# sail-sg/EditAnything

Hardware: NVIDIA H100
Metric: 512x512 50-step SAM+ControlNet-inpaint images/sec; fused ControlNetx2+UNet+CFG+DDIM step ms (higher is better)
Workload: dtype fp16 storage / fp32 accumulate

## Files before the change

### editanything_b200/csrc/ea_gemm.cu

```cuda
#include "ea_common.cuh"
#include "ea_internal.h"

namespace ea {

static constexpr int BM = 128;
static constexpr int BK = 64;
static constexpr int GEMM_THREADS = 288;
static constexpr int W_TMA = 8;
static constexpr int EPI_WARPS = 8, EPI_THREADS = 256;
static constexpr int GEMM_SMEM_RING = 216 * 1024;
__host__ __device__ constexpr int gemm_epi_bytes(int bn) { return BM * (bn + 4) * 4 + 2 * 4096 * EPI_WARPS; }
__host__ __device__ constexpr int gemm_region_bytes(int bn, int stages) {
  return stages * (BM * BK * 2 + bn * BK * 2) > gemm_epi_bytes(bn) ? stages * (BM * BK * 2 + bn * BK * 2)
                                                                    : gemm_epi_bytes(bn);
}

struct GemmKParams {
  int M, N;
  int mode;
  int nkb_main;
  int nkb_extra;
  int cin_blocks;
  int BN, stages;
  int H, W, Bsz;
  int bw, bh, bn;
  int tiles_w, tiles_h;
  const float* bias;
  const float* rowvec;
  int rows_per_batch;
  int rowvec_ld;
  const ea_half* residual;
  long long ldr;
  ea_half* out;
  long long ldo;
  ea_half* out2;
  long long ldo2;
  float* out_f32;
  int act;
  float out_scale;
  int accumulate;
  int splits;
  int kb_per_split;
  int no_spin;
  float* ws;
  int* cnt;
  float2* rowstats_out;
  const float2* ln_stats;
  const float* ln_g;
  int ln_parts;
  float ln_inv_c, ln_eps;
  const float* row_scale;
  const char* pf[EA_GEMM_MAX_PREFETCH];
  long long pf_bytes[EA_GEMM_MAX_PREFETCH];
  int pf_ctas;
  unsigned long long b_policy;
};

static constexpr int GEMM_MAX_GROUPS = 3;
struct GemmGroup {
  CUtensorMap tmA0, tmA1, tmA2, tmA3, tmAx, tmB;
  GemmKParams p;
};
template <int NG>
struct GemmLaunch {
  GemmGroup g[NG];
};

__device__ __forceinline__ void tile_origin(const GemmKParams& p, int tm, int& n0, int& h0,
                                            int& w0) {
  int per_blk = p.tiles_w * p.tiles_h;
  int nb = tm / per_blk;
  int r = tm - nb * per_blk;
  int th = r / p.tiles_w;
  n0 = nb * p.bn;
  h0 = th * p.bh;
  w0 = (r - th * p.tiles_w) * p.bw;
}

struct RowInfo {
  long long m;
  bool ok;
  int batch;
};

__device__ __forceinline__ RowInfo row_info(const GemmKParams& p, int tm, int r) {
  RowInfo ri;
  if (p.mode == EA_GEMM_LINEAR) {
    ri.m = (long long)tm * BM + r;
    ri.ok = ri.m < p.M;
    ri.batch = p.rows_per_batch > 0 ? (int)(ri.m / p.rows_per_batch) : 0;
  } else {
    int n0, h0, w0;
    tile_origin(p, tm, n0, h0, w0);
    int dn = r / (p.bw * p.bh);
    int rr = r - dn * (p.bw * p.bh);
    int dh = rr / p.bw;
    int dw = rr - dh * p.bw;
    int n = n0 + dn, h = h0 + dh, w = w0 + dw;
    ri.ok = (n < p.Bsz) && (h < p.H) && (w < p.W);
    ri.m = ((long long)n * p.H + h) * p.W + w;
    ri.batch = n;
  }
  return ri;
}

__device__ __forceinline__ void epi_bar_sync() { asm volatile("bar.sync 1, 256;" ::: "memory"); }

__device__ __forceinline__ int ld_acquire_gpu(const int* p) {
  int v;
  asm volatile("ld.acquire.gpu.global.s32 %0, [%1];" : "=r"(v) : "l"(p) : "memory");
  return v;
}

__device__ __forceinline__ void l2_prefetch_hint(const GemmKParams& p, int cta, int lane, int lane0) {
  if (cta >= p.pf_ctas || lane < lane0) return;
  const int nl = 32 - lane0;
#pragma unroll 1
  for (int i = 0; i < EA_GEMM_MAX_PREFETCH; ++i) {
    if (p.pf[i] == nullptr) continue;
    const long long nlines = p.pf_bytes[i] >> 7;
    const char* base = p.pf[i];
#pragma unroll 4
    for (long long c = (long long)cta * nl + (lane - lane0); c < nlines; c += (long long)p.pf_ctas * nl)
      asm volatile("prefetch.global.L2 [%0];" ::"l"(base + (c << 7)));
  }
}

__device__ __forceinline__ void ln_row_stats(const GemmKParams& p, long long m, float& ln_r, float& ln_nm) {
  float s = 0.f, q = 0.f;
  const float2* base = p.ln_stats + m;
  for (int j0 = 0; j0 < p.ln_parts; j0 += 16) {
    float2 v[16];
#pragma unroll
    for (int u = 0; u < 16; ++u)
      v[u] = (j0 + u < p.ln_parts) ? __ldcg(base + (size_t)(j0 + u) * p.M) : make_float2(0.f, 0.f);
#pragma unroll
    for (int u = 0; u < 16; ++u) {
      s += v[u].x;
      q += v[u].y;
    }
  }
  const float mu = s * p.ln_inv_c;
  ln_r = rsqrtf(fmaxf(q * p.ln_inv_c - mu * mu, 0.f) + p.ln_eps);
  ln_nm = -ln_r * mu;
}

__device__ __noinline__ float act_call(float x, int act) {
  return act == EA_ACT_SILU ? silu_f(x) : gelu_erf_f(x);
}

__device__ __forceinline__ void stage_put32(uint4* stg, int lane, int half, const uint4 (&o)[4]) {
#pragma unroll
  for (int q = 0; q < 4; ++q) stg[lane * 8 + ((half * 4 + q) ^ (lane & 7))] = o[q];
}
__device__ __forceinline__ void stage_flush(const uint4* stg, int lane, ea_half* out, long long ldo,
                                            ea_half* out2, long long ldo2, long long m_mine, bool ok_mine,
                                            int col0, int pieces, int n_limit, long long lin_m0, int M) {
  __syncwarp();
  const int piece = lane & 7, rsub = lane >> 3;
  const int col = col0 + piece * 8;
  const bool col_ok = piece < pieces && col < n_limit;
  uint4 val[8];
#pragma unroll
  for (int i = 0; i < 8; ++i) {
    const int row = i * 4 + rsub;
    val[i] = stg[row * 8 + (piece ^ (row & 7))];
  }
  if (lin_m0 >= 0) {
    const long long m0 = lin_m0 + rsub;
    ea_half* ptr = out + m0 * ldo + col;
    ea_half* ptr2 = out2 ? out2 + m0 * ldo2 + col : nullptr;
    const long long step = 4 * ldo, step2 = 4 * ldo2;
#pragma unroll
    for (int i = 0; i < 8; ++i) {
      if (col_ok && m0 + 4 * i < M) {
        *reinterpret_cast<uint4*>(ptr) = val[i];
        if (ptr2) *reinterpret_cast<uint4*>(ptr2) = val[i];
      }
      ptr += step;
      if (ptr2) ptr2 += step2;
    }
  } else {
#pragma unroll
    for (int i = 0; i < 8; ++i) {
      const int row = i * 4 + rsub;
      const long long m_r = __shfl_sync(0xffffffffu, m_mine, row);
      const int ok_r = __shfl_sync(0xffffffffu, (int)ok_mine, row);
      if (ok_r && col_ok) {
        *reinterpret_cast<uint4*>(out + m_r * ldo + col) = val[i];
        if (out2) *reinterpret_cast<uint4*>(out2 + m_r * ldo2 + col) = val[i];
      }
    }
  }
  __syncwarp();
}

__device__ __forceinline__ void stage_flush32(const uint4* stg, int lane, ea_half* out, long long ldo, int col0,
                                              int n_limit, long long lin_m0, int M) {
  __syncwarp();
  const int piece = lane & 3, rsub = lane >> 2;
  const int col = col0 + piece * 8;
  const bool col_ok = col < n_limit;
  uint4 val[4];
#pragma unroll
  for (int i = 0; i < 4; ++i) {
    const int row = i * 8 + rsub;
    val[i] = stg[row * 8 + (piece ^ (row & 7))];
  }
  const long long m0 = lin_m0 + rsub;
  ea_half* ptr = out + m0 * ldo + col;
  const long long step = 8 * ldo;
#pragma unroll
  for (int i = 0; i < 4; ++i) {
    if (col_ok && m0 + 8 * i < M) *reinterpret_cast<uint4*>(ptr) = val[i];
    ptr += step;
  }
  __syncwarp();
}

__device__ __forceinline__ void residual_load64(uint4 (&rr)[8], const ea_half* residual, long long ldr,
                                                int lane, long long m_mine, bool ok_mine, int col0,
                                                int cols_left, int n_limit, long long lin_m0, int M) {
  const int piece = lane & 7, rsub = lane >> 3;
  const int col = col0 + piece * 8;
#pragma unroll
  for (int i = 0; i < 8; ++i) {
    const int row = i * 4 + rsub;
    long long m_r;
    int ok_r;
    if (lin_m0 >= 0) {
      m_r = lin_m0 + row;
      ok_r = m_r < M;
    } else {
      m_r = __shfl_sync(0xffffffffu, m_mine, row);
      ok_r = __shfl_sync(0xffffffffu, (int)ok_mine, row);
    }
    rr[i] = (ok_r && piece * 8 < cols_left && col < n_limit)
                ? __ldg(reinterpret_cast<const uint4*>(residual + m_r * ldr + col))
                : make_uint4(0, 0, 0, 0);
  }
}

__device__ __forceinline__ void epilogue_geglu32(const float* cb, int half_bn, int c, float (&fx)[32],
                                                 float (&fg)[32], uint4 (&o)[4], bool ln, float ln_r,
                                                 float ln_nm) {
  uint32_t packed[16];
#pragma unroll
  for (int j = 0; j < 32; j += 4) {
    float4 bx = *reinterpret_cast<const float4*>(cb + c + j);
    float4 bg = *reinterpret_cast<const float4*>(cb + half_bn + c + j);
    if (ln) {
      const float4 gx = *reinterpret_cast<const float4*>(cb + 256 + c + j);
      const float4 gg = *reinterpret_cast<const float4*>(cb + 256 + half_bn + c + j);
      bx.x = fmaf(ln_nm, gx.x, bx.x); bx.y = fmaf(ln_nm, gx.y, bx.y); bx.z = fmaf(ln_nm, gx.z, bx.z); bx.w = fmaf(ln_nm, gx.w, bx.w);
      bg.x = fmaf(ln_nm, gg.x, bg.x); bg.y = fmaf(ln_nm, gg.y, bg.y); bg.z = fmaf(ln_nm, gg.z, bg.z); bg.w = fmaf(ln_nm, gg.w, bg.w);
    }
    const float x0 = fmaf(fx[j], ln_r, bx.x), x1 = fmaf(fx[j + 1], ln_r, bx.y);
    const float x2 = fmaf(fx[j + 2], ln_r, bx.z), x3 = fmaf(fx[j + 3], ln_r, bx.w);
    const float g0 = fmaf(fg[j], ln_r, bg.x), g1 = fmaf(fg[j + 1], ln_r, bg.y);
    const float g2 = fmaf(fg[j + 2], ln_r, bg.z), g3 = fmaf(fg[j + 3], ln_r, bg.w);
    packed[j >> 1] = ea_pack2(x0 * gelu_erf_f(g0), x1 * gelu_erf_f(g1));
    packed[(j >> 1) + 1] = ea_pack2(x2 * gelu_erf_f(g2), x3 * gelu_erf_f(g3));
  }
#pragma unroll
  for (int q = 0; q < 4; ++q)
    o[q] = make_uint4(packed[4 * q], packed[4 * q + 1], packed[4 * q + 2], packed[4 * q + 3]);
}

__device__ __forceinline__ void epilogue_geglu32_direct(const GemmKParams& p, const RowInfo& ri, int ncol0,
                                                        int half_bn, int c, float (&fx)[32],
                                                        float (&fg)[32]) {
  const int nout0 = (ncol0 >> 1) + c;
  if (!(ri.ok && nout0 < (p.N >> 1))) return;
  uint32_t packed[16];
#pragma unroll
  for (int j = 0; j < 32; j += 2) {
    float x0 = fx[j], x1 = fx[j + 1], g0 = fg[j], g1 = fg[j + 1];
    if (p.bias) {
      x0 += __ldg(p.bias + ncol0 + c + j);
      x1 += __ldg(p.bias + ncol0 + c + j + 1);
      g0 += __ldg(p.bias + ncol0 + half_bn + c + j);
      g1 += __ldg(p.bias + ncol0 + half_bn + c + j + 1);
    }
    packed[j >> 1] = ea_pack2(x0 * act_call(g0, EA_ACT_GELU), x1 * act_call(g1, EA_ACT_GELU));
  }
  uint4* dst = reinterpret_cast<uint4*>(p.out + ri.m * p.ldo + nout0);
#pragma unroll
  for (int q = 0; q < 4; ++q)
    dst[q] = make_uint4(packed[4 * q], packed[4 * q + 1], packed[4 * q + 2], packed[4 * q + 3]);
}

__device__ __forceinline__ void epilogue_chunk32(const GemmKParams& p, const RowInfo& ri,
                                                 int n_first, float (&f)[32]) {
  if (!(ri.ok && n_first < p.N)) return;
  const long long m = ri.m;
  if (p.bias) {
#pragma unroll
    for (int j = 0; j < 32; j += 4) {
      if (n_first + j < p.N) {
        float4 b = __ldg(reinterpret_cast<const float4*>(p.bias + n_first + j));
        f[j] += b.x; f[j + 1] += b.y; f[j + 2] += b.z; f[j + 3] += b.w;
      }
    }
  }
  if (p.rowvec) {
    const float* rv = p.rowvec + (long long)ri.batch * p.rowvec_ld + n_first;
#pragma unroll
    for (int j = 0; j < 32; j += 4) {
      if (n_first + j < p.N) {
        float4 b = __ldg(reinterpret_cast<const float4*>(rv + j));
        f[j] += b.x; f[j + 1] += b.y; f[j + 2] += b.z; f[j + 3] += b.w;
      }
    }
  }
  if (p.act == EA_ACT_SILU) {
#pragma unroll
    for (int j = 0; j < 32; ++j) f[j] = act_call(f[j], EA_ACT_SILU);
  } else if (p.act == EA_ACT_GELU) {
#pragma unroll
    for (int j = 0; j < 32; ++j) f[j] = act_call(f[j], EA_ACT_GELU);
  }
  if (p.out_scale != 1.0f) {
#pragma unroll
    for (int j = 0; j < 32; ++j) f[j] *= p.out_scale;
  }
  if (p.row_scale) {
    const float rs = __ldg(p.row_scale + m);
#pragma unroll
    for (int j = 0; j < 32; ++j) f[j] *= rs;
  }
  if (p.residual) {
    const uint4* rp = reinterpret_cast<const uint4*>(p.residual + m * p.ldr + n_first);
#pragma unroll
    for (int q = 0; q < 4; ++q) {
      if (n_first + q * 8 < p.N) {
        uint4 u = __ldg(rp + q);
        float2 a = ea_unpack2(u.x), b = ea_unpack2(u.y), cc = ea_unpack2(u.z), d = ea_unpack2(u.w);
        f[q * 8 + 0] += a.x; f[q * 8 + 1] += a.y; f[q * 8 + 2] += b.x; f[q * 8 + 3] += b.y;
        f[q * 8 + 4] += cc.x; f[q * 8 + 5] += cc.y; f[q * 8 + 6] += d.x; f[q * 8 + 7] += d.y;
      }
    }
  }
  if (p.out_f32) {
    float* dst = p.out_f32 + m * p.ldo + n_first;
#pragma unroll
    for (int j = 0; j < 32; j += 4) {
      if (n_first + j < p.N) {
        float4 o = make_float4(f[j], f[j + 1], f[j + 2], f[j + 3]);
        if (p.accumulate) {
          float4 old = *reinterpret_cast<float4*>(dst + j);
          o.x += old.x; o.y += old.y; o.z += old.z; o.w += old.w;
        }
        *reinterpret_cast<float4*>(dst + j) = o;
      }
    }
    return;
  }
  uint4* dst = reinterpret_cast<uint4*>(p.out + m * p.ldo + n_first);
  if (p.accumulate) {
#pragma unroll
    for (int q = 0; q < 4; ++q) {
      if (n_first + q * 8 < p.N) {
        uint4 u = dst[q];
        float2 a = ea_unpack2(u.x), b = ea_unpack2(u.y), cc = ea_unpack2(u.z), d = ea_unpack2(u.w);
        f[q * 8 + 0] += a.x; f[q * 8 + 1] += a.y; f[q * 8 + 2] += b.x; f[q * 8 + 3] += b.y;
        f[q * 8 + 4] += cc.x; f[q * 8 + 5] += cc.y; f[q * 8 + 6] += d.x; f[q * 8 + 7] += d.y;
      }
    }
  }
  uint4* dst2 = p.out2 ? reinterpret_cast<uint4*>(p.out2 + m * p.ldo2 + n_first) : nullptr;
#pragma unroll
  for (int q = 0; q < 4; ++q) {
    if (n_first + q * 8 < p.N) {
      uint4 o = make_uint4(ea_pack2(f[q * 8 + 0], f[q * 8 + 1]), ea_pack2(f[q * 8 + 2], f[q * 8 + 3]),
                           ea_pack2(f[q * 8 + 4], f[q * 8 + 5]), ea_pack2(f[q * 8 + 6], f[q * 8 + 7]));
      dst[q] = o;
      if (dst2) dst2[q] = o;
    }
  }
}


static int encode_2d(CUtensorMap* m, const void* base, uint64_t inner, uint64_t outer,
                     uint64_t row_stride_bytes, uint32_t box_inner, uint32_t box_outer) {
  cuuint64_t dims[2] = {inner, outer};
  cuuint64_t strides[1] = {row_stride_bytes};
  cuuint32_t box[2] = {box_inner, box_outer};
  cuuint32_t estr[2] = {1, 1};
  CUresult r = ea_tmap_encode()(m, EA_TMAP_DTYPE, 2, const_cast<void*>(base), dims, strides, box,
                                estr, CU_TENSOR_MAP_INTERLEAVE_NONE, CU_TENSOR_MAP_SWIZZLE_128B,
                                CU_TENSOR_MAP_L2_PROMOTION_L2_256B,
                                CU_TENSOR_MAP_FLOAT_OOB_FILL_NONE);
  return r == CUDA_SUCCESS ? 0 : (int)r;
}

static int encode_4d(CUtensorMap* m, const void* base, const uint64_t dims_[4],
                     const uint64_t strides_bytes[3], const uint32_t box_[4]) {
  cuuint64_t dims[4] = {dims_[0], dims_[1], dims_[2], dims_[3]};
  cuuint64_t strides[3] = {strides_bytes[0], strides_bytes[1], strides_bytes[2]};
  cuuint32_t box[4] = {box_[0], box_[1], box_[2], box_[3]};
  cuuint32_t estr[4] = {1, 1, 1, 1};
  CUresult r = ea_tmap_encode()(m, EA_TMAP_DTYPE, 4, const_cast<void*>(base), dims, strides, box,
                                estr, CU_TENSOR_MAP_INTERLEAVE_NONE, CU_TENSOR_MAP_SWIZZLE_128B,
                                CU_TENSOR_MAP_L2_PROMOTION_L2_256B,
                                CU_TENSOR_MAP_FLOAT_OOB_FILL_NONE);
  return r == CUDA_SUCCESS ? 0 : (int)r;
}

static void conv_geometry(int H, int W, int& bw, int& bh, int& bn) {
  bw = 1;
  while (bw * 2 <= W && bw * 2 <= 128 && (W % (bw * 2)) == 0) bw *= 2;
  bh = 1;
  while (bh * 2 <= H && bw * bh * 2 <= 128 && (H % (bh * 2)) == 0) bh *= 2;
  bn = 128 / (bw * bh);
}

__device__ __forceinline__ void acc_ld32(const float* accs, int ld, int r, int c, uint32_t (&v)[32]) {
  const float4* src = reinterpret_cast<const float4*>(accs + (size_t)r * ld + c);
#pragma unroll
  for (int j = 0; j < 8; ++j) {
    const float4 f = src[j];
    v[4 * j] = __float_as_uint(f.x); v[4 * j + 1] = __float_as_uint(f.y);
    v[4 * j + 2] = __float_as_uint(f.z); v[4 * j + 3] = __float_as_uint(f.w);
  }
}

#define EA_GEMM_TILE()                                                             \
  const int gi = NG == 1 ? 0 : tile / tiles_per_group;                             \
  const int gtile = NG == 1 ? tile : tile - gi * tiles_per_group;                  \
  const int zsplit = gtile / mn_tiles;                                             \
  const int mn = gtile - zsplit * mn_tiles;                                        \
  const GemmGroup& GG = L.g[gi];                                                   \
  const GemmKParams& p = GG.p;                                                     \
  const int tm = mn % m_tiles, tn = mn / m_tiles;                                  \
  const int kb0 = zsplit * p.kb_per_split;                                         \
  const int kb1 = min(nkb, kb0 + p.kb_per_split);

template <int BN, int NG>
__global__ void __launch_bounds__(GEMM_THREADS, 1)
ea_gemm_kernel(const __grid_constant__ GemmLaunch<NG> L, const int tiles_per_group, const int m_tiles,
               const int n_groups) {
  const GemmKParams& p0 = L.g[0].p;
  const int n_tiles = (p0.N + BN - 1) / BN;
  const int mn_tiles = m_tiles * n_tiles;
  const int num_tiles = tiles_per_group * (NG == 1 ? 1 : n_groups);
  const int nkb = p0.nkb_main + p0.nkb_extra;
  constexpr int a_bytes = BM * BK * 2;
  constexpr int stage_bytes = a_bytes + BN * BK * 2;
  constexpr int ACC_LD = BN + 4;
  extern __shared__ __align__(1024) uint8_t smem_raw[];
  uint8_t* smem = reinterpret_cast<uint8_t*>((reinterpret_cast<uintptr_t>(smem_raw) + 1023) &
                                             ~uintptr_t(1023));
  float* accs = reinterpret_cast<float*>(smem);
  uint8_t* stg_base = smem + BM * ACC_LD * 4;
  uint64_t* full_bar = reinterpret_cast<uint64_t*>(smem + gemm_region_bytes(BN, p0.stages));
  uint64_t* empty_bar = full_bar + p0.stages;
  uint64_t* epi_done = empty_bar + p0.stages;
  float* cb = reinterpret_cast<float*>(epi_done + 2);

  pdl_launch_dependents();
  const int warp = threadIdx.x >> 5;
  const int lane = threadIdx.x & 31;

  if (warp == W_TMA && lane == 0) {
    const int g0 = NG == 1 ? 0 : min((int)blockIdx.x / tiles_per_group, n_groups - 1);
    tma_prefetch_desc(&L.g[g0].tmA0);
    tma_prefetch_desc(&L.g[g0].tmB);
    if (p0.mode == EA_GEMM_CONV_S2 || p0.mode == EA_GEMM_CONV_S2A) {
      tma_prefetch_desc(&L.g[g0].tmA1);
      tma_prefetch_desc(&L.g[g0].tmA2);
      tma_prefetch_desc(&L.g[g0].tmA3);
    }
    if (p0.nkb_extra > 0) tma_prefetch_desc(&L.g[g0].tmAx);
  }
  if (warp == W_TMA) {
    for (int g = 0; g < (NG == 1 ? 1 : n_groups); ++g) l2_prefetch_hint(L.g[g].p, (int)blockIdx.x, lane, 2);
  }
  if (warp == W_TMA && lane == 1) {
    for (int s = 0; s < p0.stages; ++s) {
      mbar_init(&full_bar[s], 1);
      mbar_init(&empty_bar[s], EPI_WARPS);
    }
    mbar_init(epi_done, EPI_WARPS);
    fence_mbar_init();
  }
  __syncthreads();

  if (warp >= EPI_WARPS) {
    pdl_wait();
    if (lane != 0) return;
    int stage = 0;
    uint32_t phase = 0;
    uint8_t* sa = smem;
    int it = 0;
    for (int tile = blockIdx.x; tile < num_tiles; tile += gridDim.x, ++it) {
      EA_GEMM_TILE()
      const CUtensorMap& tmA0 = GG.tmA0;
      const CUtensorMap& tmA1 = GG.tmA1;
      const CUtensorMap& tmA2 = GG.tmA2;
      const CUtensorMap& tmA3 = GG.tmA3;
      const CUtensorMap& tmAx = GG.tmAx;
      const CUtensorMap& tmB = GG.tmB;
      if (it > 0) mbar_wait(epi_done, (uint32_t)((it - 1) & 1));
      const int bcol = tn * BN;
      if (p.mode == EA_GEMM_LINEAR) {
        const int arow = tm * BM;
        for (int kb = kb0; kb < kb1; ++kb) {
          mbar_wait(&empty_bar[stage], phase ^ 1u);
          mbar_expect_tx(&full_bar[stage], (uint32_t)stage_bytes);
          tma_load_2d(sa, &tmA0, &full_bar[stage], kb * BK, arow);
          tma_load_2d_hint(sa + a_bytes, &tmB, &full_bar[stage], kb * BK, bcol, p.b_policy);
          sa += stage_bytes;
          if (++stage == p.stages) { stage = 0; phase ^= 1u; sa = smem; }
        }
      } else {
        int n0, h0, w0;
        tile_origin(p, tm, n0, h0, w0);
        int tap = kb0 / p.cin_blocks;
        int c0 = (kb0 - tap * p.cin_blocks) * BK;
        int kh = tap / 3, kw = tap - kh * 3;
        const int cin = p.cin_blocks * BK;
        for (int kb = kb0; kb < kb1; ++kb) {
          mbar_wait(&empty_bar[stage], phase ^ 1u);
          mbar_expect_tx(&full_bar[stage], (uint32_t)stage_bytes);
          if (kb >= p.nkb_main) {
            tma_load_4d(sa, &tmAx, &full_bar[stage], (kb - p.nkb_main) * BK, w0, h0, n0);
          } else if (p.mode == EA_GEMM_CONV_S1) {
            tma_load_4d(sa, &tmA0, &full_bar[stage], c0, w0 + kw - 1, h0 + kh - 1, n0);
          } else {
            const bool asym = p.mode == EA_GEMM_CONV_S2A;
            const int ph = asym ? (kh == 1 ? 1 : 0) : (kh == 1 ? 0 : 1);
            const int dh = asym ? (kh == 2 ? 1 : 0) : (kh == 0 ? -1 : 0);
            const int pw = asym ? (kw == 1 ? 1 : 0) : (kw == 1 ? 0 : 1);
            const int dw = asym ? (kw == 2 ? 1 : 0) : (kw == 0 ? -1 : 0);
            const int sel = ph * 2 + pw;
            const CUtensorMap* m = sel == 0 ? &tmA0 : sel == 1 ? &tmA1 : sel == 2 ? &tmA2 : &tmA3;
            tma_load_4d(sa, m, &full_bar[stage], c0, w0 + dw, h0 + dh, n0);
          }
          tma_load_2d_hint(sa + a_bytes, &tmB, &full_bar[stage], kb * BK, bcol, p.b_policy);
          c0 += BK;
          if (c0 == cin) { c0 = 0; if (++kw == 3) { kw = 0; ++kh; } }
          sa += stage_bytes;
          if (++stage == p.stages) { stage = 0; phase ^= 1u; sa = smem; }
        }
      }
    }
    return;
  }

  pdl_wait();
  const int wg = warp >> 2;
  const int wq = warp & 3;
  const int r = wq * 32 + lane;
  const int et = threadIdx.x;
  constexpr int GSTEP = 128;
  uint4* stg = reinterpret_cast<uint4*>(stg_base + warp * 4096);
  uint4* stg2 = reinterpret_cast<uint4*>(stg_base + 4096 * EPI_WARPS + warp * 4096);
  const uint32_t smem0 = smem_u32(smem);
  int stage = 0;
  uint32_t phase = 0;
  int it = 0;
  for (int tile = blockIdx.x; tile < num_tiles; tile += gridDim.x, ++it) {
    EA_GEMM_TILE()
    const bool geglu = p.act == EA_ACT_GEGLU;
    const int half_bn = BN >> 1;
    const bool has_res = p.residual != nullptr;
    const RowInfo ri = row_info(p, tm, r);
    const int ncol0 = tn * BN;
    float* cbt = cb + (it & 1) * 512;
    const long long lin_m0 = p.mode == EA_GEMM_LINEAR ? (long long)tm * BM + wq * 32 : -1;
    const int b_first = row_info(p, tm, 0).batch, b_last = row_info(p, tm, BM - 1).batch;
    const bool fast = p.splits == 1 && !geglu && !p.out_f32 && !p.accumulate && !p.row_scale && (b_last - b_first) <= 1;
    uint4 rres[8];
    const bool ln = p.ln_stats != nullptr;
    float ln_r = 1.f, ln_nm = 0.f;
    if (ln && ri.ok) ln_row_stats(p, ri.m, ln_r, ln_nm);
    if (fast) {
      for (int i = et; i < BN; i += EPI_THREADS) {
        const int col = ncol0 + i;
        float v0 = 0.f, v1 = 0.f;
        if (col < p.N) {
          const float bsum = p.bias ? __ldg(p.bias + col) : 0.f;
          v0 = bsum + (p.rowvec ? __ldg(p.rowvec + (long long)b_first * p.rowvec_ld + col) : 0.f);
          v1 = ln ? __ldg(p.ln_g + col)
                  : bsum + (p.rowvec ? __ldg(p.rowvec + (long long)b_last * p.rowvec_ld + col) : 0.f);
        }
        cbt[i] = v0;
        cbt[256 + i] = v1;
      }
      if (has_res && wg * 64 < BN)
        residual_load64(rres, p.residual, p.ldr, lane, ri.m, ri.ok, ncol0 + wg * 64, BN - wg * 64, p.N, lin_m0, p.M);
    } else if (geglu && p.splits == 1) {
      for (int i = et; i < BN; i += EPI_THREADS) {
        const bool in = ncol0 + i < p.N;
        cbt[i] = (p.bias && in) ? __ldg(p.bias + ncol0 + i) : 0.f;
        if (ln) cbt[256 + i] = in ? __ldg(p.ln_g + ncol0 + i) : 0.f;
      }
    }

    {
      float acc[BN / 2];
#pragma unroll
      for (int i = 0; i < BN / 2; ++i) acc[i] = 0.f;
      int prev = -1;
      for (int kb = kb0; kb < kb1; ++kb) {
        mbar_wait(&full_bar[stage], phase);
        const uint32_t sa = smem0 + (uint32_t)(stage * stage_bytes);
        const uint64_t da = gmma_desc_k_sw128(sa + (uint32_t)(wg * 64 * 128), 1024);
        const uint64_t db = gmma_desc_k_sw128(sa + (uint32_t)a_bytes, 1024);
        wgmma_fence();
#pragma unroll
        for (int k = 0; k < 4; ++k) Wgmma<BN>::ss(acc, da + 2 * k, db + 2 * k, 1u);
        wgmma_commit();
        wgmma_wait<1>();
        if (prev >= 0) {
          __syncwarp();
          if (lane == 0) mbar_arrive(&empty_bar[prev]);
        }
        prev = stage;
        if (++stage == p.stages) { stage = 0; phase ^= 1u; }
      }
      wgmma_wait<0>();
      wgmma_fence_regs(acc);
      if (prev >= 0) {
        __syncwarp();
        if (lane == 0) mbar_arrive(&empty_bar[prev]);
      }
      epi_bar_sync();
      const int r0 = wg * 64 + wq * 16 + (lane >> 2);
      float* d0 = accs + (size_t)r0 * ACC_LD + 2 * (lane & 3);
#pragma unroll
      for (int j = 0; j < BN / 8; ++j) {
        *reinterpret_cast<float2*>(d0 + 8 * j) = make_float2(acc[4 * j], acc[4 * j + 1]);
        *reinterpret_cast<float2*>(d0 + 8 * ACC_LD + 8 * j) = make_float2(acc[4 * j + 2], acc[4 * j + 3]);
      }
    }
    epi_bar_sync();

    if (fast) {
      const float* cbr = cbt + ((!ln && ri.batch != b_first) ? 256 : 0);
      auto next_chunk = [&](int c) { return ((c & 32) == 0 && c + 32 < BN) ? c + 32 : (c & ~63) + GSTEP; };
      for (int c = wg * 64; c < BN; c = next_chunk(c)) {
        uint32_t v[32];
        acc_ld32(accs, ACC_LD, r, c, v);
        const int n_first = ncol0 + c;
        const int half = (c >> 5) & 1;
        if (has_res && half == 0) {
          const int piece = lane & 7, rsub = lane >> 3;
#pragma unroll
          for (int i = 0; i < 8; ++i) {
            const int row = i * 4 + rsub;
            stg2[row * 8 + (piece ^ (row & 7))] = rres[i];
          }
          __syncwarp();
          if (c + GSTEP < BN)
            residual_load64(rres, p.residual, p.ldr, lane, ri.m, ri.ok, n_first + GSTEP, BN - c - GSTEP, p.N, lin_m0, p.M);
        }
        float f[32];
        if (ln) {
#pragma unroll
          for (int j = 0; j < 32; j += 4) {
            const float4 b4 = *reinterpret_cast<const float4*>(cbt + c + j);
            const float4 g4 = *reinterpret_cast<const float4*>(cbt + 256 + c + j);
            f[j] = fmaf(__uint_as_float(v[j]), ln_r, fmaf(ln_nm, g4.x, b4.x));
            f[j + 1] = fmaf(__uint_as_float(v[j + 1]), ln_r, fmaf(ln_nm, g4.y, b4.y));
            f[j + 2] = fmaf(__uint_as_float(v[j + 2]), ln_r, fmaf(ln_nm, g4.z, b4.z));
            f[j + 3] = fmaf(__uint_as_float(v[j + 3]), ln_r, fmaf(ln_nm, g4.w, b4.w));
          }
        } else {
#pragma unroll
          for (int j = 0; j < 32; j += 4) {
            const float4 b4 = *reinterpret_cast<const float4*>(cbr + c + j);
            f[j] = __uint_as_float(v[j]) + b4.x;
            f[j + 1] = __uint_as_float(v[j + 1]) + b4.y;
            f[j + 2] = __uint_as_float(v[j + 2]) + b4.z;
            f[j + 3] = __uint_as_float(v[j + 3]) + b4.w;
          }
        }
        if (p.act == EA_ACT_SILU) {
#pragma unroll
          for (int j = 0; j < 32; ++j) f[j] = act_call(f[j], EA_ACT_SILU);
        } else if (p.act == EA_ACT_GELU) {
#pragma unroll
          for (int j = 0; j < 32; ++j) f[j] = gelu_erf_f(f[j]);
        }
        if (p.out_scale != 1.0f) {
#pragma unroll
          for (int j = 0; j < 32; ++j) f[j] *= p.out_scale;
        }
#pragma unroll
        for (int q = 0; q < 4; ++q) {
          const int slot = lane * 8 + ((half * 4 + q) ^ (lane & 7));
          if (has_res) {
            const uint4 rc = stg2[slot];
            const float2 a = ea_unpack2(rc.x), b = ea_unpack2(rc.y), cc = ea_unpack2(rc.z), d = ea_unpack2(rc.w);
            f[q * 8 + 0] += a.x; f[q * 8 + 1] += a.y; f[q * 8 + 2] += b.x; f[q * 8 + 3] += b.y;
            f[q * 8 + 4] += cc.x; f[q * 8 + 5] += cc.y; f[q * 8 + 6] += d.x; f[q * 8 + 7] += d.y;
          }
          stg[slot] = make_uint4(ea_pack2(f[q * 8 + 0], f[q * 8 + 1]), ea_pack2(f[q * 8 + 2], f[q * 8 + 3]),
                                 ea_pack2(f[q * 8 + 4], f[q * 8 + 5]), ea_pack2(f[q * 8 + 6], f[q * 8 + 7]));
        }
        if (p.rowstats_out) {
          float s0 = 0.f, s1 = 0.f, q0 = 0.f, q1 = 0.f;
#pragma unroll
          for (int j = 0; j < 32; j += 2) {
            s0 += f[j]; q0 = fmaf(f[j], f[j], q0);
            s1 += f[j + 1]; q1 = fmaf(f[j + 1], f[j + 1], q1);
          }
          if (ri.ok && n_first < p.N) p.rowstats_out[(size_t)(n_first >> 5) * p.M + ri.m] = make_float2(s0 + s1, q0 + q1);
        }
        if (half == 1 || c + 32 >= BN)
          stage_flush(stg, lane, p.out, p.ldo, p.out2, p.ldo2, ri.m, ri.ok, n_first - half * 32,
                      half == 1 ? 8 : 4, p.N, lin_m0, p.M);
      }
    } else if (p.splits == 1) {
      if (geglu) {
        for (int c = wg * 32; c < half_bn; c += 64) {
          uint32_t xv[32], gv[32];
          acc_ld32(accs, ACC_LD, r, c, xv);
          acc_ld32(accs, ACC_LD, r, half_bn + c, gv);
          float fx[32], fg[32];
#pragma unroll
          for (int j = 0; j < 32; ++j) { fx[j] = __uint_as_float(xv[j]); fg[j] = __uint_as_float(gv[j]); }
          uint4 o[4];
          epilogue_geglu32(cbt, half_bn, c, fx, fg, o, ln, ln_r, ln_nm);
          stage_put32(stg, lane, 0, o);
          if (lin_m0 >= 0)
            stage_flush32(stg, lane, p.out, p.ldo, (ncol0 >> 1) + c, p.N >> 1, lin_m0, p.M);
          else
            stage_flush(stg, lane, p.out, p.ldo, nullptr, 0, ri.m, ri.ok, (ncol0 >> 1) + c, 4, p.N >> 1, lin_m0, p.M);
        }
      } else {
        for (int c = wg * 32; c < BN; c += 64) {
          uint32_t v[32];
          acc_ld32(accs, ACC_LD, r, c, v);
          float f[32];
#pragma unroll
          for (int j = 0; j < 32; ++j) f[j] = __uint_as_float(v[j]);
          epilogue_chunk32(p, ri, ncol0 + c, f);
          __syncwarp();
        }
      }
    } else {
      const int tile_id = tn * m_tiles + tm;
      float* wtile = p.ws + (size_t)tile_id * p.splits * (BM * BN);
      float* mine = wtile + (size_t)zsplit * (BM * BN);
      for (int c = wg * 32; c < BN; c += 64) {
        uint32_t v[32];
        acc_ld32(accs, ACC_LD, r, c, v);
        float4* dst = reinterpret_cast<float4*>(mine + (size_t)r * BN + c);
#pragma unroll
        for (int j = 0; j < 8; ++j)
          __stcg(dst + j, make_float4(__uint_as_float(v[4 * j]), __uint_as_float(v[4 * j + 1]),
                                      __uint_as_float(v[4 * j + 2]), __uint_as_float(v[4 * j + 3])));
      }
      __threadfence();
      epi_bar_sync();
      int* cnt = p.cnt + 2 * tile_id;
      bool take_all = false;
      volatile int* flag = reinterpret_cast<volatile int*>(cbt);
      if (p.no_spin) {
        if (et == 0) *flag = atomicAdd(cnt, 1);
        epi_bar_sync();
        take_all = *flag == p.splits - 1;
        epi_bar_sync();
      } else {
        if (et == 0) {
          atomicAdd(cnt, 1);
          uint32_t spins = 0;
          while (ld_acquire_gpu(cnt) < p.splits) {
            __nanosleep(40);
            if (++spins > (1u << 24)) { asm volatile("trap;"); }
          }
        }
        epi_bar_sync();
      }
      __threadfence();
      if (!p.no_spin || take_all) {
        const int chunks = geglu ? (half_bn >> 5) : (BN >> 5);
        const int units = BM * chunks;
        const int u0 = take_all ? 0 : (int)(((long long)units * zsplit) / p.splits);
        const int u1 = take_all ? units : (int)(((long long)units * (zsplit + 1)) / p.splits);
        const int segs = geglu ? 2 : 1;
        const int ustride = segs * 32 + 4;
        float* stage_f = accs;
        const size_t split_stride = (size_t)BM * BN;
        for (int ub = u0; ub < u1; ub += EPI_THREADS) {
          const int nu = min(EPI_THREADS, u1 - ub);
          const int nvec4 = nu * segs * 8;
          for (int idx = et; idx < nvec4; idx += EPI_THREADS) {
            const int ul = idx / (segs * 8);
            const int rem = idx - ul * (segs * 8);
            const int seg = rem >> 3, q = rem & 7;
            const int u = ub + ul;
            const int rr = u & (BM - 1);
            const int c = ((u >> 7) << 5) + seg * half_bn * (geglu ? 1 : 0);
            const float4* src = reinterpret_cast<const float4*>(wtile + (size_t)rr * BN + c) + q;
            float4 acc = make_float4(0.f, 0.f, 0.f, 0.f);
            int sidx = 0;
            for (; sidx + 4 <= p.splits; sidx += 4) {
              float4 v0 = __ldcg(src + (size_t)(sidx + 0) * (split_stride >> 2));
              float4 v1 = __ldcg(src + (size_t)(sidx + 1) * (split_stride >> 2));
              float4 v2 = __ldcg(src + (size_t)(sidx + 2) * (split_stride >> 2));
              float4 v3 = __ldcg(src + (size_t)(sidx + 3) * (split_stride >> 2));
              acc.x += v0.x; acc.y += v0.y; acc.z += v0.z; acc.w += v0.w;
              acc.x += v1.x; acc.y += v1.y; acc.z += v1.z; acc.w += v1.w;
              acc.x += v2.x; acc.y += v2.y; acc.z += v2.z; acc.w += v2.w;
              acc.x += v3.x; acc.y += v3.y; acc.z += v3.z; acc.w += v3.w;
            }
            for (; sidx < p.splits; ++sidx) {
              float4 v0 = __ldcg(src + (size_t)sidx * (split_stride >> 2));
              acc.x += v0.x; acc.y += v0.y; acc.z += v0.z; acc.w += v0.w;
            }
            *reinterpret_cast<float4*>(stage_f + ul * ustride + seg * 32 + q * 4) = acc;
          }
          epi_bar_sync();
          if (et < nu) {
            const int u = ub + et;
            const int rr = u & (BM - 1);
            const int c = (u >> 7) << 5;
            RowInfo r2 = row_info(p, tm, rr);
            const float4* sp = reinterpret_cast<const float4*>(stage_f + et * ustride);
            float f[32];
#pragma unroll
            for (int j = 0; j < 8; ++j) {
              float4 v = sp[j];
              f[4 * j] = v.x; f[4 * j + 1] = v.y; f[4 * j + 2] = v.z; f[4 * j + 3] = v.w;
            }
            if (geglu) {
              float fg[32];
#pragma unroll
              for (int j = 0; j < 8; ++j) {
                float4 v = sp[8 + j];
                fg[4 * j] = v.x; fg[4 * j + 1] = v.y; fg[4 * j + 2] = v.z; fg[4 * j + 3] = v.w;
              }
              epilogue_geglu32_direct(p, r2, ncol0, half_bn, c, f, fg);
            } else {
              epilogue_chunk32(p, r2, ncol0 + c, f);
            }
          }
          epi_bar_sync();
        }
        epi_bar_sync();
        if (et == 0) {
          if (take_all) {
            cnt[0] = 0;
          } else {
            int old = atomicAdd(cnt + 1, 1);
            if (old == p.splits - 1) {
              cnt[0] = 0;
              cnt[1] = 0;
            }
          }
        }
      }
    }
    fence_proxy_async();
    __syncwarp();
    if (lane == 0) mbar_arrive(epi_done);
  }
}
#undef EA_GEMM_TILE

struct GemmPlan { int BN, stages, splits, kbps, occ; double cost; };

static constexpr double PL_LAT = 2100.0, PL_SM_CAP = 57.0, PL_L2 = 3000.0, PL_HBM = 1900.0;
static constexpr double PL_SPLIT_COL = 8.0, PL_SPLIT_FIX = 7000.0;
static constexpr double PL_START = 3800.0, PL_EPI = 50.0, PL_EPI_RES = 21.0;
static constexpr int GEMM_BN[3] = {128, 64, 32};

static GemmPlan plan_gemm(int mt, int N, int nkb, int act, long long ws_floats, int n_sm, bool has_res = false,
                          int groups = 1) {
  const double epi_col = (PL_EPI + (has_res ? PL_EPI_RES : 0.0)) * (act == EA_ACT_GEGLU ? 0.84 : 1.0);
  GemmPlan best = {0, 0, 1, nkb, 1, 1e30};
  for (int BN : GEMM_BN) {
    if (act == EA_ACT_GEGLU && BN != 128) continue;
    if (BN > 32 && N <= BN - 32) continue;
    const int nt = (N + BN - 1) / BN;
    const long long tiles = (long long)mt * nt * groups;
    const int stage_bytes = BM * BK * 2 + BN * BK * 2;
    int st = GEMM_SMEM_RING / stage_bytes;
    if (st > 8) st = 8;
    if (st > nkb) st = nkb < 2 ? 2 : nkb;
    const long long slots = n_sm;
    for (int pass = 0; pass < 2; ++pass) {
      int splits = 1, kbps = nkb;
      if (pass == 1) {
        if (tiles >= slots || nkb < 8) break;
        int s_max = (int)(slots / tiles);
        if (s_max > nkb / 4) s_max = nkb / 4;
        if (s_max < 2) break;
        kbps = (nkb + s_max - 1) / s_max;
        splits = (nkb + kbps - 1) / kbps;
        if (splits < 2) break;
        if (tiles > 2048 || tiles * splits * (long long)(BM * BN) > ws_floats) break;
      }
      const long long ctas = tiles * splits;
      const long long waves = (ctas + slots - 1) / slots;
      const long long conc = ctas < slots ? ctas : slots;
      const double t_mma = 4.0 * BN;
      const double t_sm = (double)stage_bytes / PL_SM_CAP;
      const double a_bytes = BM * BK * 2.0, b_bytes = BN * BK * 2.0;
      const double hbm_frac = 1.0 / (double)mt;
      const double t_chip = (double)conc * (a_bytes / PL_L2 + b_bytes * hbm_frac / PL_HBM +
                                            b_bytes * (1.0 - hbm_frac) / PL_L2);
      const double t_lat = PL_LAT / st;
      double t_kb = t_mma;
      if (t_sm > t_kb) t_kb = t_sm;
      if (t_chip > t_kb) t_kb = t_chip;
      if (t_lat > t_kb) t_kb = t_lat;
      double cost;
      if (splits == 1) {
        cost = (double)waves * (PL_START + kbps * t_kb + epi_col * BN);
      } else {
        cost = (double)waves * (PL_START + kbps * t_kb + PL_SPLIT_COL * BN) + PL_SPLIT_FIX +
               3.0 * (BM * BN * 4.0) / 25.0 + 150.0 * splits;
      }
      if (cost < best.cost) best = {BN, st, splits, kbps, 1, cost};
    }
  }
  return best;
}

static int sm_count() { return ea_sm_count(); }

}

using namespace ea;

extern "C" int ea_gemm_plan(int m_tiles, int N, int k_blocks, int act, long long workspace_bytes,
                            int n_sm, int* out5) {
  if (!out5 || m_tiles <= 0 || N <= 0 || k_blocks <= 0) return EA_ERR_ARG;
  const long long ws_floats = workspace_bytes > 65536 ? (workspace_bytes - 65536) / 4 : 0;
  GemmPlan pl = plan_gemm(m_tiles, N, k_blocks, act, ws_floats, n_sm > 0 ? n_sm : 132);
  out5[0] = pl.BN; out5[1] = pl.stages; out5[2] = pl.splits; out5[3] = pl.kbps;
  out5[4] = pl.occ;
  return pl.BN ? EA_OK : EA_ERR_SHAPE;
}

struct GemmShape {
  int m_tiles, nkb;
  long long Ktot;
  bool ln_any;
};

static int gemm_fill_group(const ea_gemm_args* a, GemmGroup& G, GemmShape& sh) {
  if (!a || !a->a || !a->w || (!a->out && !a->out_f32)) return EA_ERR_ARG;
  if (a->mode < 0 || a->mode > EA_GEMM_CONV_S2A) return EA_ERR_ARG;
  if (a->N <= 0 || a->M <= 0) return EA_ERR_ARG;
  if (a->N % 8 != 0) return EA_ERR_SHAPE;
  GemmKParams& p = G.p;
  memset(&p, 0, sizeof(p));
  p.M = a->M;
  p.N = a->N;
  p.mode = a->mode;
  p.bias = a->bias;
  p.rowvec = a->rowvec;
  p.rows_per_batch = a->rows_per_batch;
  p.rowvec_ld = a->rowvec_ld;
  p.residual = reinterpret_cast<const ea_half*>(a->residual);
  p.ldr = a->ldr;
  p.out = reinterpret_cast<ea_half*>(a->out);
  p.ldo = a->ldo;
  p.out2 = reinterpret_cast<ea_half*>(a->out2);
  p.ldo2 = a->ldo2;
  p.out_f32 = a->out_f32;
  p.act = a->act;
  p.out_scale = a->out_scale;
  p.accumulate = a->accumulate;
  p.row_scale = a->row_scale;
  for (int i = 0; i < EA_GEMM_MAX_PREFETCH; ++i) {
    p.pf[i] = reinterpret_cast<const char*>(a->prefetch[i]);
    p.pf_bytes[i] = a->prefetch[i] ? (a->prefetch_bytes[i] & ~15LL) : 0;
  }
  p.pf_ctas = 0;
  p.b_policy = 0x12F0000000000000ull;
  if (a->row_scale && (a->act == EA_ACT_GEGLU || a->rowstats_out || a->ln_stats)) return EA_ERR_ARG;
  sh.ln_any = a->rowstats_out || a->ln_stats;
  if (sh.ln_any) {
    if (a->mode != EA_GEMM_LINEAR || a->rowvec || a->out_f32 || a->accumulate) return EA_ERR_ARG;
    if (a->rowstats_out && (a->N % 32 != 0 || a->act == EA_ACT_GEGLU)) return EA_ERR_SHAPE;
    if (a->ln_stats && (!a->ln_g || a->ln_parts <= 0 || a->K != a->ln_parts * 32)) return EA_ERR_ARG;
    p.rowstats_out = reinterpret_cast<float2*>(a->rowstats_out);
    p.ln_stats = reinterpret_cast<const float2*>(a->ln_stats);
    p.ln_g = a->ln_g;
    p.ln_parts = a->ln_parts;
    p.ln_inv_c = a->ln_stats ? 1.0f / (float)a->K : 0.f;
    p.ln_eps = a->ln_eps;
  }
  if (p.ldo % 8 != 0 || (p.residual && p.ldr % 8 != 0) || (p.out2 && p.ldo2 % 8 != 0))
    return EA_ERR_SHAPE;

  CUtensorMap* tmA[4] = {&G.tmA0, &G.tmA1, &G.tmA2, &G.tmA3};
  if (a->mode == EA_GEMM_LINEAR) {
    if (a->K % 8 != 0 || a->lda % 8 != 0) return EA_ERR_SHAPE;
    p.nkb_main = (a->K + BK - 1) / BK;
    p.nkb_extra = 0;
    p.cin_blocks = 1;
    sh.m_tiles = (a->M + BM - 1) / BM;
    sh.Ktot = a->K;
    if (encode_2d(tmA[0], a->a, (uint64_t)a->K, (uint64_t)a->M, (uint64_t)a->lda * 2, BK, BM))
      return EA_ERR_TMAP;
    G.tmA1 = G.tmA2 = G.tmA3 = G.tmA0;
    G.tmAx = G.tmA0;
  } else {
    const int H = a->H, W = a->W, B = a->Bsz, C = a->Cin;
    if (C % 64 != 0 || H <= 0 || W <= 0 || B <= 0) return EA_ERR_SHAPE;
    if ((long long)B * H * W != a->M) return EA_ERR_SHAPE;
    p.H = H; p.W = W; p.Bsz = B;
    conv_geometry(H, W, p.bw, p.bh, p.bn);
    p.tiles_w = W / p.bw;
    p.tiles_h = H / p.bh;
    p.cin_blocks = C / 64;
    p.nkb_main = 9 * p.cin_blocks;
    p.nkb_extra = 0;
    sh.m_tiles = ((B + p.bn - 1) / p.bn) * p.tiles_w * p.tiles_h;
    sh.Ktot = 9LL * C;
    const long long lda = a->lda > 0 ? a->lda : C;
    uint32_t box[4] = {64, (uint32_t)p.bw, (uint32_t)p.bh, (uint32_t)p.bn};
    if (a->mode == EA_GEMM_CONV_S1) {
      uint64_t dims[4] = {(uint64_t)C, (uint64_t)W, (uint64_t)H, (uint64_t)B};
      uint64_t st[3] = {(uint64_t)lda * 2, (uint64_t)lda * W * 2, (uint64_t)lda * W * H * 2};
      if (encode_4d(tmA[0], a->a, dims, st, box)) return EA_ERR_TMAP;
      G.tmA1 = G.tmA2 = G.tmA3 = G.tmA0;
    } else {
      const int Hin = 2 * H, Win = 2 * W;
      for (int ph = 0; ph < 2; ++ph)
        for (int pw = 0; pw < 2; ++pw) {
          const ea_half* base =
              reinterpret_cast<const ea_half*>(a->a) + ((long long)ph * Win + pw) * lda;
          uint64_t dims[4] = {(uint64_t)C, (uint64_t)W, (uint64_t)H, (uint64_t)B};
          uint64_t st[3] = {(uint64_t)lda * 2 * 2, (uint64_t)lda * Win * 2 * 2,
                            (uint64_t)lda * Win * Hin * 2};
          if (encode_4d(tmA[ph * 2 + pw], base, dims, st, box)) return EA_ERR_TMAP;
        }
    }
    G.tmAx = G.tmA0;
    if (a->a_extra) {
      if (a->mode != EA_GEMM_CONV_S1 || a->Cin_extra % 64 != 0) return EA_ERR_SHAPE;
      const long long ldx = a->ld_extra > 0 ? a->ld_extra : a->Cin_extra;
      uint64_t dims[4] = {(uint64_t)a->Cin_extra, (uint64_t)W, (uint64_t)H, (uint64_t)B};
      uint64_t st[3] = {(uint64_t)ldx * 2, (uint64_t)ldx * W * 2, (uint64_t)ldx * W * H * 2};
      if (encode_4d(&G.tmAx, a->a_extra, dims, st, box)) return EA_ERR_TMAP;
      p.nkb_extra = a->Cin_extra / 64;
      sh.Ktot += a->Cin_extra;
    }
  }
  sh.nkb = p.nkb_main + p.nkb_extra;
  return EA_OK;
}

static bool gemm_same_problem(const ea_gemm_args* a, const ea_gemm_args* b) {
  return a->mode == b->mode && a->M == b->M && a->N == b->N && a->K == b->K && a->Bsz == b->Bsz && a->H == b->H &&
         a->W == b->W && a->Cin == b->Cin && a->Cin_extra == b->Cin_extra && (!a->a_extra) == (!b->a_extra) &&
         a->act == b->act && a->accumulate == b->accumulate && (!a->out_f32) == (!b->out_f32) &&
         (!a->row_scale) == (!b->row_scale) &&
         (!a->rowvec) == (!b->rowvec) && a->rows_per_batch == b->rows_per_batch &&
         (!a->rowstats_out) == (!b->rowstats_out) && (!a->ln_stats) == (!b->ln_stats) && a->ln_parts == b->ln_parts &&
         a->force_bn == b->force_bn && a->force_stages == b->force_stages && a->force_splits == b->force_splits &&
         a->force_2cta == b->force_2cta && a->no_spin == b->no_spin && a->force_persistent == b->force_persistent;
}

template <typename K>
static int set_max_smem(K kernel, int bytes, int& cached) {
  if (bytes > cached) {
    const cudaError_t e = cudaFuncSetAttribute(kernel, cudaFuncAttributeMaxDynamicSharedMemorySize, bytes);
    if (e != cudaSuccess) return ea_cuda_fail(e, "ea_gemm: cudaFuncSetAttribute(MaxDynamicSharedMemorySize)");
    cached = bytes;
  }
  return EA_OK;
}

template <int BN, int NG>
static cudaError_t launch_gemm(const GemmLaunch<NG>& L, int grid, int smem_bytes, int tiles_per_group, int m_tiles,
                               int n_groups, cudaStream_t stream, int& rc) {
  static int cache[EA_MAX_DEV];
  if ((rc = set_max_smem(ea_gemm_kernel<BN, NG>, smem_bytes, cache[ea_dev()]))) return cudaSuccess;
  return ea_launch(ea_gemm_kernel<BN, NG>, dim3((unsigned)grid), dim3(GEMM_THREADS), (size_t)smem_bytes, stream, L,
                   tiles_per_group, m_tiles, n_groups);
}

template <int NG>
static cudaError_t launch_gemm_bn(int BN, const GemmLaunch<NG>& L, int grid, int smem_bytes, int tiles_per_group,
                                  int m_tiles, int n_groups, cudaStream_t stream, int& rc) {
  switch (BN) {
    case 32: return launch_gemm<32, NG>(L, grid, smem_bytes, tiles_per_group, m_tiles, n_groups, stream, rc);
    case 64: return launch_gemm<64, NG>(L, grid, smem_bytes, tiles_per_group, m_tiles, n_groups, stream, rc);
    case 128: return launch_gemm<128, NG>(L, grid, smem_bytes, tiles_per_group, m_tiles, n_groups, stream, rc);
    default: return launch_gemm<256, NG>(L, grid, smem_bytes, tiles_per_group, m_tiles, n_groups, stream, rc);
  }
}

extern "C" int ea_gemm_grouped(const ea_gemm_args* args, int n_groups, void* stream_) {
  cudaStream_t stream = reinterpret_cast<cudaStream_t>(stream_);
  if (!args || n_groups < 1 || n_groups > GEMM_MAX_GROUPS) return EA_ERR_ARG;
  const ea_gemm_args* a = &args[0];
  static GemmLaunch<GEMM_MAX_GROUPS> L;
  GemmShape sh0;
  memset(&L, 0, sizeof(L));
  for (int g = 0; g < n_groups; ++g) {
    GemmShape shg;
    if (g > 0 && !gemm_same_problem(a, &args[g])) return EA_ERR_ARG;
    const int rc = gemm_fill_group(&args[g], L.g[g], g == 0 ? sh0 : shg);
    if (rc != EA_OK) return rc;
  }
  const int m_tiles = sh0.m_tiles, nkb = sh0.nkb;
  const bool ln_any = sh0.ln_any;
  const int G = n_groups;
  const long long ws_floats =
      (a->workspace && a->workspace_bytes > 65536 && !ln_any) ? (a->workspace_bytes - 65536) / 4 : 0;
  const bool persist = a->force_persistent > 0;
  const bool has_res = a->residual != nullptr;
  GemmPlan plan = plan_gemm(m_tiles, a->N, nkb, a->act, persist ? 0 : ws_floats, sm_count(), has_res, G);
  if (a->force_bn > 0 || a->force_stages > 0 || a->force_splits > 0) {
    if (a->force_bn > 0) plan.BN = a->force_bn;
    const int sb = BM * BK * 2 + plan.BN * BK * 2;
    if (a->force_bn > 0) plan.stages = plan.BN <= 128 ? 3 : 4;
    if (a->force_stages > 0) plan.stages = a->force_stages;
    if (plan.stages * sb > GEMM_SMEM_RING) plan.stages = GEMM_SMEM_RING / sb;
    if (plan.stages > nkb) plan.stages = nkb < 2 ? 2 : nkb;
    if (a->force_bn > 0 || a->force_splits > 0) { plan.splits = 1; plan.kbps = nkb; }
    if (a->force_splits > 1 && !persist) {
      plan.kbps = (nkb + a->force_splits - 1) / a->force_splits;
      plan.splits = (nkb + plan.kbps - 1) / plan.kbps;
    }
  }
  if (ln_any && plan.splits > 1) return EA_ERR_ARG;
  const int BN = plan.BN;
  if (BN != 32 && BN != 64 && BN != 128 && BN != 256) return EA_ERR_SHAPE;
  if (a->act == EA_ACT_GEGLU && (a->N % 128 != 0 || BN != 128)) return EA_ERR_SHAPE;
  const int n_tiles = (a->N + BN - 1) / BN;
  const long long tiles = (long long)m_tiles * n_tiles;
  if (plan.splits > 1 &&
      (!ws_floats || tiles * G > 8192 || tiles * G * plan.splits * (long long)(BM * BN) > ws_floats))
    return EA_ERR_SHAPE;
  if (plan.splits > 1 && !a->no_spin && tiles * G * plan.splits > (long long)sm_count()) return EA_ERR_SHAPE;

  int stages = plan.stages;
  if (stages > 8) stages = 8;
  if (stages < 2) stages = 2;
  const int smem_bytes = gemm_region_bytes(BN, stages) + (2 * stages + 2) * 8 + 2 * 2 * 256 * 4 + 1024;
  const long long tiles_per_group = tiles * plan.splits;
  for (int g = 0; g < G; ++g) {
    GemmKParams& p = L.g[g].p;
    const ea_gemm_args* ag = &args[g];
    p.BN = BN;
    p.stages = stages;
    p.splits = plan.splits;
    p.kb_per_split = plan.kbps;
    p.no_spin = a->no_spin;
    if (p.splits > 1) {
      p.cnt = reinterpret_cast<int*>(a->workspace) + 2 * g * tiles;
      p.ws = reinterpret_cast<float*>(reinterpret_cast<char*>(a->workspace) + 65536) +
             (size_t)g * tiles * p.splits * (BM * BN);
    }
    const long long ldw = ag->ldw > 0 ? ag->ldw : sh0.Ktot;
    if (ldw % 8 != 0) return EA_ERR_SHAPE;
    if (encode_2d(&L.g[g].tmB, ag->w, (uint64_t)sh0.Ktot, (uint64_t)ag->N, (uint64_t)ldw * 2, BK, (uint32_t)BN))
      return EA_ERR_TMAP;
  }
  if (m_tiles > 64)
    for (int g = 0; g < G; ++g) L.g[g].p.b_policy = 0ull;
  const long long total = tiles_per_group * G;
  const int grid = (int)(persist && total > sm_count() ? sm_count() : total);
  for (int g = 0; g < G; ++g)
    L.g[g].p.pf_ctas = grid < sm_count() ? grid : sm_count();

  cudaError_t le;
  int rc = EA_OK;
  if (G == 1) {
    GemmLaunch<1> L1;
    L1.g[0] = L.g[0];
    le = launch_gemm_bn<1>(BN, L1, grid, smem_bytes, (int)tiles_per_group, m_tiles, G, stream, rc);
  } else {
    le = launch_gemm_bn<GEMM_MAX_GROUPS>(BN, L, grid, smem_bytes, (int)tiles_per_group, m_tiles, G, stream, rc);
  }
  if (rc) return rc;
  ea_count_launch();
  if (le != cudaSuccess) return ea_cuda_fail(le, "ea_gemm: kernel launch");
  const cudaError_t ke = cudaGetLastError();
  return ke == cudaSuccess ? 0 : ea_cuda_fail(ke, "ea_gemm: after the kernel launch");
}

extern "C" int ea_gemm(const ea_gemm_args* a, void* stream) { return ea_gemm_grouped(a, 1, stream); }
```

Measured before the change: 1.618.

## Warp-specialize GEMM with separate MMA and epilogue warpgroups and register rebalancing

Splits the GEMM kernel into a producer warp, dedicated MMA warps and separate epilogue warps, so the epilogue of one tile can overlap the mainloop of the next. Accumulator staging moves to its own shared-memory region with acc_full/acc_empty barriers, and setmaxnreg redistributes registers between roles. Small-BN and short-K tiles also default to a persistent grid. The cost is fewer pipeline stages, because the ring and the epilogue buffer now share shared memory, plus more threads per CTA, which can cost registers in the MMA warps.

```diff
diff --git a/editanything_b200/csrc/ea_gemm.cu b/editanything_b200/csrc/ea_gemm.cu
--- a/editanything_b200/csrc/ea_gemm.cu
+++ b/editanything_b200/csrc/ea_gemm.cu
@@ -5,14 +5,43 @@
 
 static constexpr int BM = 128;
 static constexpr int BK = 64;
-static constexpr int GEMM_THREADS = 288;
-static constexpr int W_TMA = 8;
+static constexpr int GEMM_THREADS = 640;
+static constexpr int W_TMA = 16;
+static constexpr int MMA_WARPS = 8;
 static constexpr int EPI_WARPS = 8, EPI_THREADS = 256;
+static constexpr int GEMM_LAUNCH_REGS = (65536 / GEMM_THREADS) & ~7;
+template <int BN, bool SPLIT>
+struct GemmRegs {
+  static constexpr bool split_epi = SPLIT;
+  static constexpr int producer = 48;
+  static constexpr int mma = split_epi ? BN / 2 + 32 : 192;
+  static constexpr int epi = split_epi ? ((5 * GEMM_LAUNCH_REGS - producer - 2 * mma) / 2) & ~7 : 24;
+  static_assert(producer + 2 * mma + 2 * epi <= 5 * GEMM_LAUNCH_REGS, "setmaxnreg budgets exceed the launch");
+};
+template <int R> __device__ __forceinline__ void setmaxnreg() {
+  if constexpr (R > GEMM_LAUNCH_REGS)
+    asm volatile("setmaxnreg.inc.sync.aligned.u32 %0;" ::"n"(R));
+  else if constexpr (R < GEMM_LAUNCH_REGS)
+    asm volatile("setmaxnreg.dec.sync.aligned.u32 %0;" ::"n"(R));
+}
 static constexpr int GEMM_SMEM_RING = 216 * 1024;
-__host__ __device__ constexpr int gemm_epi_bytes(int bn) { return BM * (bn + 4) * 4 + 2 * 4096 * EPI_WARPS; }
-__host__ __device__ constexpr int gemm_region_bytes(int bn, int stages) {
-  return stages * (BM * BK * 2 + bn * BK * 2) > gemm_epi_bytes(bn) ? stages * (BM * BK * 2 + bn * BK * 2)
-                                                                    : gemm_epi_bytes(bn);
+static constexpr int GEMM_SMEM_MAX = 227 * 1024;
+__host__ __device__ constexpr int gemm_epi_bytes(int bn) { return BM * (bn + 4) * 4 + 4096 * EPI_WARPS; }
+__host__ __device__ constexpr int gemm_ring_bytes(int bn, int stages) { return stages * (BM * BK * 2 + bn * BK * 2); }
+__host__ __device__ constexpr int gemm_region_bytes(int bn, int stages, bool split) {
+  return split ? gemm_ring_bytes(bn, stages) + gemm_epi_bytes(bn)
+               : (gemm_ring_bytes(bn, stages) > gemm_epi_bytes(bn) ? gemm_ring_bytes(bn, stages) : gemm_epi_bytes(bn));
+}
+__host__ __device__ constexpr int gemm_smem_bytes(int bn, int stages, bool split) {
+  return gemm_region_bytes(bn, stages, split) + (2 * stages + 2) * 8 + 2 * 2 * 256 * 4 + 1024;
+}
+static constexpr int GEMM_SPLIT_EPI_MAX_KB = 20;
+static bool gemm_split_epi(int bn, int kb_per_tile, int splits) {
+  return bn < 128 || (bn == 128 && splits == 1 && kb_per_tile <= GEMM_SPLIT_EPI_MAX_KB);
+}
+static int gemm_fit_stages(int bn, int stages, bool split) {
+  while (stages > 2 && gemm_smem_bytes(bn, stages, split) > GEMM_SMEM_MAX) --stages;
+  return stages;
 }
 
 struct GemmKParams {
@@ -436,10 +465,276 @@
   const int kb0 = zsplit * p.kb_per_split;                                         \
   const int kb1 = min(nkb, kb0 + p.kb_per_split);
 
-template <int BN, int NG>
+template <int BN, typename AccReady>
+__device__ __forceinline__ void gemm_epilogue(const GemmKParams& p, int tm, int tn, int zsplit, int m_tiles,
+                                              float* cbt, float* accs, uint4* stg, int wg, int wq, int lane, int et,
+                                              AccReady&& acc_ready) {
+  constexpr int ACC_LD = BN + 4;
+  const int r = wq * 32 + lane;
+  constexpr int GSTEP = 128;
+  const bool geglu = p.act == EA_ACT_GEGLU;
+  const int half_bn = BN >> 1;
+  const bool has_res = p.residual != nullptr;
+  const RowInfo ri = row_info(p, tm, r);
+  const int ncol0 = tn * BN;
+  const long long lin_m0 = p.mode == EA_GEMM_LINEAR ? (long long)tm * BM + wq * 32 : -1;
+  const int b_first = row_info(p, tm, 0).batch, b_last = row_info(p, tm, BM - 1).batch;
+  const bool fast = p.splits == 1 && !geglu && !p.out_f32 && !p.accumulate && !p.row_scale && (b_last - b_first) <= 1;
+  uint4 rres[8];
+  const bool ln = p.ln_stats != nullptr;
+  float ln_r = 1.f, ln_nm = 0.f;
+  if (ln && ri.ok) ln_row_stats(p, ri.m, ln_r, ln_nm);
+  if (fast) {
+    for (int i = et; i < BN; i += EPI_THREADS) {
+      const int col = ncol0 + i;
+      float v0 = 0.f, v1 = 0.f;
+      if (col < p.N) {
+        const float bsum = p.bias ? __ldg(p.bias + col) : 0.f;
+        v0 = bsum + (p.rowvec ? __ldg(p.rowvec + (long long)b_first * p.rowvec_ld + col) : 0.f);
+        v1 = ln ? __ldg(p.ln_g + col)
+                : bsum + (p.rowvec ? __ldg(p.rowvec + (long long)b_last * p.rowvec_ld + col) : 0.f);
+      }
+      cbt[i] = v0;
+      cbt[256 + i] = v1;
+    }
+    if (has_res && wg * 64 < BN)
+      residual_load64(rres, p.residual, p.ldr, lane, ri.m, ri.ok, ncol0 + wg * 64, BN - wg * 64, p.N, lin_m0, p.M);
+  } else if (geglu && p.splits == 1) {
+    for (int i = et; i < BN; i += EPI_THREADS) {
+      const bool in = ncol0 + i < p.N;
+      cbt[i] = (p.bias && in) ? __ldg(p.bias + ncol0 + i) : 0.f;
+      if (ln) cbt[256 + i] = in ? __ldg(p.ln_g + ncol0 + i) : 0.f;
+    }
+  }
+
+  acc_ready();
+  epi_bar_sync();
+
+  if (fast) {
+    const float* cbr = cbt + ((!ln && ri.batch != b_first) ? 256 : 0);
+    auto next_chunk = [&](int c) { return ((c & 32) == 0 && c + 32 < BN) ? c + 32 : (c & ~63) + GSTEP; };
+    for (int c = wg * 64; c < BN; c = next_chunk(c)) {
+      uint32_t v[32];
+      acc_ld32(accs, ACC_LD, r, c, v);
+      const int n_first = ncol0 + c;
+      const int half = (c >> 5) & 1;
+      if (has_res && half == 0) {
+        const int piece = lane & 7, rsub = lane >> 3;
+#pragma unroll
+        for (int i = 0; i < 8; ++i) {
+          const int row = i * 4 + rsub;
+          stg[row * 8 + (piece ^ (row & 7))] = rres[i];
+        }
+        __syncwarp();
+        if (c + GSTEP < BN)
+          residual_load64(rres, p.residual, p.ldr, lane, ri.m, ri.ok, n_first + GSTEP, BN - c - GSTEP, p.N, lin_m0, p.M);
+      }
+      float f[32];
+      if (ln) {
+#pragma unroll
+        for (int j = 0; j < 32; j += 4) {
+          const float4 b4 = *reinterpret_cast<const float4*>(cbt + c + j);
+          const float4 g4 = *reinterpret_cast<const float4*>(cbt + 256 + c + j);
+          f[j] = fmaf(__uint_as_float(v[j]), ln_r, fmaf(ln_nm, g4.x, b4.x));
+          f[j + 1] = fmaf(__uint_as_float(v[j + 1]), ln_r, fmaf(ln_nm, g4.y, b4.y));
+          f[j + 2] = fmaf(__uint_as_float(v[j + 2]), ln_r, fmaf(ln_nm, g4.z, b4.z));
+          f[j + 3] = fmaf(__uint_as_float(v[j + 3]), ln_r, fmaf(ln_nm, g4.w, b4.w));
+        }
+      } else {
+#pragma unroll
+        for (int j = 0; j < 32; j += 4) {
+          const float4 b4 = *reinterpret_cast<const float4*>(cbr + c + j);
+          f[j] = __uint_as_float(v[j]) + b4.x;
+          f[j + 1] = __uint_as_float(v[j + 1]) + b4.y;
+          f[j + 2] = __uint_as_float(v[j + 2]) + b4.z;
+          f[j + 3] = __uint_as_float(v[j + 3]) + b4.w;
+        }
+      }
+      if (p.act == EA_ACT_SILU) {
+#pragma unroll
+        for (int j = 0; j < 32; ++j) f[j] = act_call(f[j], EA_ACT_SILU);
+      } else if (p.act == EA_ACT_GELU) {
+#pragma unroll
+        for (int j = 0; j < 32; ++j) f[j] = gelu_erf_f(f[j]);
+      }
+      if (p.out_scale != 1.0f) {
+#pragma unroll
+        for (int j = 0; j < 32; ++j) f[j] *= p.out_scale;
+      }
+#pragma unroll
+      for (int q = 0; q < 4; ++q) {
+        const int slot = lane * 8 + ((half * 4 + q) ^ (lane & 7));
+        if (has_res) {
+          const uint4 rc = stg[slot];
+          const float2 a = ea_unpack2(rc.x), b = ea_unpack2(rc.y), cc = ea_unpack2(rc.z), d = ea_unpack2(rc.w);
+          f[q * 8 + 0] += a.x; f[q * 8 + 1] += a.y; f[q * 8 + 2] += b.x; f[q * 8 + 3] += b.y;
+          f[q * 8 + 4] += cc.x; f[q * 8 + 5] += cc.y; f[q * 8 + 6] += d.x; f[q * 8 + 7] += d.y;
+        }
+        stg[slot] = make_uint4(ea_pack2(f[q * 8 + 0], f[q * 8 + 1]), ea_pack2(f[q * 8 + 2], f[q * 8 + 3]),
+                               ea_pack2(f[q * 8 + 4], f[q * 8 + 5]), ea_pack2(f[q * 8 + 6], f[q * 8 + 7]));
+      }
+      if (p.rowstats_out) {
+        float s0 = 0.f, s1 = 0.f, q0 = 0.f, q1 = 0.f;
+#pragma unroll
+        for (int j = 0; j < 32; j += 2) {
+          s0 += f[j]; q0 = fmaf(f[j], f[j], q0);
+          s1 += f[j + 1]; q1 = fmaf(f[j + 1], f[j + 1], q1);
+        }
+        if (ri.ok && n_first < p.N) p.rowstats_out[(size_t)(n_first >> 5) * p.M + ri.m] = make_float2(s0 + s1, q0 + q1);
+      }
+      if (half == 1 || c + 32 >= BN)
+        stage_flush(stg, lane, p.out, p.ldo, p.out2, p.ldo2, ri.m, ri.ok, n_first - half * 32,
+                    half == 1 ? 8 : 4, p.N, lin_m0, p.M);
+    }
+  } else if (p.splits == 1) {
+    if (geglu) {
+      for (int c = wg * 32; c < half_bn; c += 64) {
+        uint32_t xv[32], gv[32];
+        acc_ld32(accs, ACC_LD, r, c, xv);
+        acc_ld32(accs, ACC_LD, r, half_bn + c, gv);
+        float fx[32], fg[32];
+#pragma unroll
+        for (int j = 0; j < 32; ++j) { fx[j] = __uint_as_float(xv[j]); fg[j] = __uint_as_float(gv[j]); }
+        uint4 o[4];
+        epilogue_geglu32(cbt, half_bn, c, fx, fg, o, ln, ln_r, ln_nm);
+        stage_put32(stg, lane, 0, o);
+        if (lin_m0 >= 0)
+          stage_flush32(stg, lane, p.out, p.ldo, (ncol0 >> 1) + c, p.N >> 1, lin_m0, p.M);
+        else
+          stage_flush(stg, lane, p.out, p.ldo, nullptr, 0, ri.m, ri.ok, (ncol0 >> 1) + c, 4, p.N >> 1, lin_m0, p.M);
+      }
+    } else {
+      for (int c = wg * 32; c < BN; c += 64) {
+        uint32_t v[32];
+        acc_ld32(accs, ACC_LD, r, c, v);
+        float f[32];
+#pragma unroll
+        for (int j = 0; j < 32; ++j) f[j] = __uint_as_float(v[j]);
+        epilogue_chunk32(p, ri, ncol0 + c, f);
+        __syncwarp();
+      }
+    }
+  } else {
+    const int tile_id = tn * m_tiles + tm;
+    float* wtile = p.ws + (size_t)tile_id * p.splits * (BM * BN);
+    float* mine = wtile + (size_t)zsplit * (BM * BN);
+    for (int c = wg * 32; c < BN; c += 64) {
+      uint32_t v[32];
+      acc_ld32(accs, ACC_LD, r, c, v);
+      float4* dst = reinterpret_cast<float4*>(mine + (size_t)r * BN + c);
+#pragma unroll
+      for (int j = 0; j < 8; ++j)
+        __stcg(dst + j, make_float4(__uint_as_float(v[4 * j]), __uint_as_float(v[4 * j + 1]),
+                                    __uint_as_float(v[4 * j + 2]), __uint_as_float(v[4 * j + 3])));
+    }
+    __threadfence();
+    epi_bar_sync();
+    int* cnt = p.cnt + 2 * tile_id;
+    bool take_all = false;
+    volatile int* flag = reinterpret_cast<volatile int*>(cbt);
+    if (p.no_spin) {
+      if (et == 0) *flag = atomicAdd(cnt, 1);
+      epi_bar_sync();
+      take_all = *flag == p.splits - 1;
+      epi_bar_sync();
+    } else {
+      if (et == 0) {
+        atomicAdd(cnt, 1);
+        uint32_t spins = 0;
+        while (ld_acquire_gpu(cnt) < p.splits) {
+          __nanosleep(40);
+          if (++spins > (1u << 24)) { asm volatile("trap;"); }
+        }
+      }
+      epi_bar_sync();
+    }
+    __threadfence();
+    if (!p.no_spin || take_all) {
+      const int chunks = geglu ? (half_bn >> 5) : (BN >> 5);
+      const int units = BM * chunks;
+      const int u0 = take_all ? 0 : (int)(((long long)units * zsplit) / p.splits);
+      const int u1 = take_all ? units : (int)(((long long)units * (zsplit + 1)) / p.splits);
+      const int segs = geglu ? 2 : 1;
+      const int ustride = segs * 32 + 4;
+      float* stage_f = accs;
+      const size_t split_stride = (size_t)BM * BN;
+      for (int ub = u0; ub < u1; ub += EPI_THREADS) {
+        const int nu = min(EPI_THREADS, u1 - ub);
+        const int nvec4 = nu * segs * 8;
+        for (int idx = et; idx < nvec4; idx += EPI_THREADS) {
+          const int ul = idx / (segs * 8);
+          const int rem = idx - ul * (segs * 8);
+          const int seg = rem >> 3, q = rem & 7;
+          const int u = ub + ul;
+          const int rr = u & (BM - 1);
+          const int c = ((u >> 7) << 5) + seg * half_bn * (geglu ? 1 : 0);
+          const float4* src = reinterpret_cast<const float4*>(wtile + (size_t)rr * BN + c) + q;
+          float4 acc = make_float4(0.f, 0.f, 0.f, 0.f);
+          int sidx = 0;
+          for (; sidx + 4 <= p.splits; sidx += 4) {
+            float4 v0 = __ldcg(src + (size_t)(sidx + 0) * (split_stride >> 2));
+            float4 v1 = __ldcg(src + (size_t)(sidx + 1) * (split_stride >> 2));
+            float4 v2 = __ldcg(src + (size_t)(sidx + 2) * (split_stride >> 2));
+            float4 v3 = __ldcg(src + (size_t)(sidx + 3) * (split_stride >> 2));
+            acc.x += v0.x; acc.y += v0.y; acc.z += v0.z; acc.w += v0.w;
+            acc.x += v1.x; acc.y += v1.y; acc.z += v1.z; acc.w += v1.w;
+            acc.x += v2.x; acc.y += v2.y; acc.z += v2.z; acc.w += v2.w;
+            acc.x += v3.x; acc.y += v3.y; acc.z += v3.z; acc.w += v3.w;
+          }
+          for (; sidx < p.splits; ++sidx) {
+            float4 v0 = __ldcg(src + (size_t)sidx * (split_stride >> 2));
+            acc.x += v0.x; acc.y += v0.y; acc.z += v0.z; acc.w += v0.w;
+          }
+          *reinterpret_cast<float4*>(stage_f + ul * ustride + seg * 32 + q * 4) = acc;
+        }
+        epi_bar_sync();
+        if (et < nu) {
+          const int u = ub + et;
+          const int rr = u & (BM - 1);
+          const int c = (u >> 7) << 5;
+          RowInfo r2 = row_info(p, tm, rr);
+          const float4* sp = reinterpret_cast<const float4*>(stage_f + et * ustride);
+          float f[32];
+#pragma unroll
+          for (int j = 0; j < 8; ++j) {
+            float4 v = sp[j];
+            f[4 * j] = v.x; f[4 * j + 1] = v.y; f[4 * j + 2] = v.z; f[4 * j + 3] = v.w;
+          }
+          if (geglu) {
+            float fg[32];
+#pragma unroll
+            for (int j = 0; j < 8; ++j) {
+              float4 v = sp[8 + j];
+              fg[4 * j] = v.x; fg[4 * j + 1] = v.y; fg[4 * j + 2] = v.z; fg[4 * j + 3] = v.w;
+            }
+            epilogue_geglu32_direct(p, r2, ncol0, half_bn, c, f, fg);
+          } else {
+            epilogue_chunk32(p, r2, ncol0 + c, f);
+          }
+        }
+        epi_bar_sync();
+      }
+      epi_bar_sync();
+      if (et == 0) {
+        if (take_all) {
+          cnt[0] = 0;
+        } else {
+          int old = atomicAdd(cnt + 1, 1);
+          if (old == p.splits - 1) {
+            cnt[0] = 0;
+            cnt[1] = 0;
+          }
+        }
+      }
+    }
+  }
+}
+
+template <int BN, int NG, bool SPLIT>
 __global__ void __launch_bounds__(GEMM_THREADS, 1)
 ea_gemm_kernel(const __grid_constant__ GemmLaunch<NG> L, const int tiles_per_group, const int m_tiles,
                const int n_groups) {
+  using R = GemmRegs<BN, SPLIT>;
   const GemmKParams& p0 = L.g[0].p;
   const int n_tiles = (p0.N + BN - 1) / BN;
   const int mn_tiles = m_tiles * n_tiles;
@@ -451,12 +746,13 @@
   extern __shared__ __align__(1024) uint8_t smem_raw[];
   uint8_t* smem = reinterpret_cast<uint8_t*>((reinterpret_cast<uintptr_t>(smem_raw) + 1023) &
                                              ~uintptr_t(1023));
-  float* accs = reinterpret_cast<float*>(smem);
-  uint8_t* stg_base = smem + BM * ACC_LD * 4;
-  uint64_t* full_bar = reinterpret_cast<uint64_t*>(smem + gemm_region_bytes(BN, p0.stages));
+  float* accs = reinterpret_cast<float*>(R::split_epi ? smem + gemm_ring_bytes(BN, p0.stages) : smem);
+  uint8_t* stg_base = reinterpret_cast<uint8_t*>(accs) + BM * ACC_LD * 4;
+  uint64_t* full_bar = reinterpret_cast<uint64_t*>(smem + gemm_region_bytes(BN, p0.stages, SPLIT));
   uint64_t* empty_bar = full_bar + p0.stages;
-  uint64_t* epi_done = empty_bar + p0.stages;
-  float* cb = reinterpret_cast<float*>(epi_done + 2);
+  uint64_t* acc_full = empty_bar + p0.stages;
+  uint64_t* acc_empty = acc_full + 1;
+  float* cb = reinterpret_cast<float*>(acc_empty + 1);
 
   pdl_launch_dependents();
   const int warp = threadIdx.x >> 5;
@@ -479,16 +775,18 @@
   if (warp == W_TMA && lane == 1) {
     for (int s = 0; s < p0.stages; ++s) {
       mbar_init(&full_bar[s], 1);
-      mbar_init(&empty_bar[s], EPI_WARPS);
-    }
-    mbar_init(epi_done, EPI_WARPS);
+      mbar_init(&empty_bar[s], MMA_WARPS);
+    }
+    mbar_init(acc_full, MMA_WARPS);
+    mbar_init(acc_empty, R::split_epi ? EPI_WARPS : MMA_WARPS);
     fence_mbar_init();
   }
   __syncthreads();
 
-  if (warp >= EPI_WARPS) {
+  if (warp >= W_TMA) {
+    setmaxnreg<R::producer>();
     pdl_wait();
-    if (lane != 0) return;
+    if (warp != W_TMA || lane != 0) return;
     int stage = 0;
     uint32_t phase = 0;
     uint8_t* sa = smem;
@@ -501,7 +799,7 @@
       const CUtensorMap& tmA3 = GG.tmA3;
       const CUtensorMap& tmAx = GG.tmAx;
       const CUtensorMap& tmB = GG.tmB;
-      if (it > 0) mbar_wait(epi_done, (uint32_t)((it - 1) & 1));
+      if (!R::split_epi && it > 0) mbar_wait(acc_empty, (uint32_t)((it - 1) & 1));
       const int bcol = tn * BN;
       if (p.mode == EA_GEMM_LINEAR) {
         const int arow = tm * BM;
@@ -548,57 +846,38 @@
     return;
   }
 
+  if (warp < EPI_WARPS) {
+    if constexpr (!R::split_epi) {
+      setmaxnreg<R::epi>();
+      return;
+    } else {
+      setmaxnreg<R::epi>();
+      pdl_wait();
+      int it = 0;
+      for (int tile = blockIdx.x; tile < num_tiles; tile += gridDim.x, ++it) {
+        EA_GEMM_TILE()
+        (void)kb0; (void)kb1;
+        gemm_epilogue<BN>(p, tm, tn, zsplit, m_tiles, cb + (it & 1) * 512, accs,
+                          reinterpret_cast<uint4*>(stg_base + warp * 4096), warp >> 2, warp & 3, lane, threadIdx.x,
+                          [&] { mbar_wait(acc_full, (uint32_t)(it & 1)); });
+        __syncwarp();
+        if (lane == 0) mbar_arrive(acc_empty);
+      }
+      return;
+    }
+  }
+
+  setmaxnreg<R::mma>();
   pdl_wait();
-  const int wg = warp >> 2;
+  const int wg = (warp >> 2) - 2;
   const int wq = warp & 3;
-  const int r = wq * 32 + lane;
-  const int et = threadIdx.x;
-  constexpr int GSTEP = 128;
-  uint4* stg = reinterpret_cast<uint4*>(stg_base + warp * 4096);
-  uint4* stg2 = reinterpret_cast<uint4*>(stg_base + 4096 * EPI_WARPS + warp * 4096);
   const uint32_t smem0 = smem_u32(smem);
   int stage = 0;
   uint32_t phase = 0;
   int it = 0;
   for (int tile = blockIdx.x; tile < num_tiles; tile += gridDim.x, ++it) {
     EA_GEMM_TILE()
-    const bool geglu = p.act == EA_ACT_GEGLU;
-    const int half_bn = BN >> 1;
-    const bool has_res = p.residual != nullptr;
-    const RowInfo ri = row_info(p, tm, r);
-    const int ncol0 = tn * BN;
-    float* cbt = cb + (it & 1) * 512;
-    const long long lin_m0 = p.mode == EA_GEMM_LINEAR ? (long long)tm * BM + wq * 32 : -1;
-    const int b_first = row_info(p, tm, 0).batch, b_last = row_info(p, tm, BM - 1).batch;
-    const bool fast = p.splits == 1 && !geglu && !p.out_f32 && !p.accumulate && !p.row_scale && (b_last - b_first) <= 1;
-    uint4 rres[8];
-    const bool ln = p.ln_stats != nullptr;
-    float ln_r = 1.f, ln_nm = 0.f;
-    if (ln && ri.ok) ln_row_stats(p, ri.m, ln_r, ln_nm);
-    if (fast) {
-      for (int i = et; i < BN; i += EPI_THREADS) {
-        const int col = ncol0 + i;
-        float v0 = 0.f, v1 = 0.f;
-        if (col < p.N) {
-          const float bsum = p.bias ? __ldg(p.bias + col) : 0.f;
-          v0 = bsum + (p.rowvec ? __ldg(p.rowvec + (long long)b_first * p.rowvec_ld + col) : 0.f);
-          v1 = ln ? __ldg(p.ln_g + col)
-                  : bsum + (p.rowvec ? __ldg(p.rowvec + (long long)b_last * p.rowvec_ld + col) : 0.f);
-        }
-        cbt[i] = v0;
-        cbt[256 + i] = v1;
-      }
-      if (has_res && wg * 64 < BN)
-        residual_load64(rres, p.residual, p.ldr, lane, ri.m, ri.ok, ncol0 + wg * 64, BN - wg * 64, p.N, lin_m0, p.M);
-    } else if (geglu && p.splits == 1) {
-      for (int i = et; i < BN; i += EPI_THREADS) {
-        const bool in = ncol0 + i < p.N;
-        cbt[i] = (p.bias && in) ? __ldg(p.bias + ncol0 + i) : 0.f;
-        if (ln) cbt[256 + i] = in ? __ldg(p.ln_g + ncol0 + i) : 0.f;
-      }
-    }
-
-    {
+    auto mma_tile = [&] {
       float acc[BN / 2];
 #pragma unroll
       for (int i = 0; i < BN / 2; ++i) acc[i] = 0.f;
@@ -610,7 +889,14 @@
         const uint64_t db = gmma_desc_k_sw128(sa + (uint32_t)a_bytes, 1024);
         wgmma_fence();
 #pragma unroll
-        for (int k = 0; k < 4; ++k) Wgmma<BN>::ss(acc, da + 2 * k, db + 2 * k, 1u);
+        for (int k = 0; k < 4; ++k) {
+          if constexpr (BN == 256) {
+            Wgmma<128>::ss(*reinterpret_cast<float(*)[64]>(acc), da + 2 * k, db + 2 * k, 1u);
+            Wgmma<128>::ss(*reinterpret_cast<float(*)[64]>(acc + 64), da + 2 * k, db + (128 * 128 >> 4) + 2 * k, 1u);
+          } else {
+            Wgmma<BN>::ss(acc, da + 2 * k, db + 2 * k, 1u);
+          }
+        }
         wgmma_commit();
         wgmma_wait<1>();
         if (prev >= 0) {
@@ -626,7 +912,11 @@
         __syncwarp();
         if (lane == 0) mbar_arrive(&empty_bar[prev]);
       }
-      epi_bar_sync();
+      if constexpr (R::split_epi) {
+        mbar_wait(acc_empty, (uint32_t)((it & 1) ^ 1));
+      } else {
+        epi_bar_sync();
+      }
       const int r0 = wg * 64 + wq * 16 + (lane >> 2);
       float* d0 = accs + (size_t)r0 * ACC_LD + 2 * (lane & 3);
 #pragma unroll
@@ -634,230 +924,19 @@
         *reinterpret_cast<float2*>(d0 + 8 * j) = make_float2(acc[4 * j], acc[4 * j + 1]);
         *reinterpret_cast<float2*>(d0 + 8 * ACC_LD + 8 * j) = make_float2(acc[4 * j + 2], acc[4 * j + 3]);
       }
-    }
-    epi_bar_sync();
-
-    if (fast) {
-      const float* cbr = cbt + ((!ln && ri.batch != b_first) ? 256 : 0);
-      auto next_chunk = [&](int c) { return ((c & 32) == 0 && c + 32 < BN) ? c + 32 : (c & ~63) + GSTEP; };
-      for (int c = wg * 64; c < BN; c = next_chunk(c)) {
-        uint32_t v[32];
-        acc_ld32(accs, ACC_LD, r, c, v);
-        const int n_first = ncol0 + c;
-        const int half = (c >> 5) & 1;
-        if (has_res && half == 0) {
-          const int piece = lane & 7, rsub = lane >> 3;
-#pragma unroll
-          for (int i = 0; i < 8; ++i) {
-            const int row = i * 4 + rsub;
-            stg2[row * 8 + (piece ^ (row & 7))] = rres[i];
-          }
-          __syncwarp();
-          if (c + GSTEP < BN)
-            residual_load64(rres, p.residual, p.ldr, lane, ri.m, ri.ok, n_first + GSTEP, BN - c - GSTEP, p.N, lin_m0, p.M);
-        }
-        float f[32];
-        if (ln) {
-#pragma unroll
-          for (int j = 0; j < 32; j += 4) {
-            const float4 b4 = *reinterpret_cast<const float4*>(cbt + c + j);
-            const float4 g4 = *reinterpret_cast<const float4*>(cbt + 256 + c + j);
-            f[j] = fmaf(__uint_as_float(v[j]), ln_r, fmaf(ln_nm, g4.x, b4.x));
-            f[j + 1] = fmaf(__uint_as_float(v[j + 1]), ln_r, fmaf(ln_nm, g4.y, b4.y));
-            f[j + 2] = fmaf(__uint_as_float(v[j + 2]), ln_r, fmaf(ln_nm, g4.z, b4.z));
-            f[j + 3] = fmaf(__uint_as_float(v[j + 3]), ln_r, fmaf(ln_nm, g4.w, b4.w));
-          }
-        } else {
-#pragma unroll
-          for (int j = 0; j < 32; j += 4) {
-            const float4 b4 = *reinterpret_cast<const float4*>(cbr + c + j);
-            f[j] = __uint_as_float(v[j]) + b4.x;
-            f[j + 1] = __uint_as_float(v[j + 1]) + b4.y;
-            f[j + 2] = __uint_as_float(v[j + 2]) + b4.z;
-            f[j + 3] = __uint_as_float(v[j + 3]) + b4.w;
-          }
-        }
-        if (p.act == EA_ACT_SILU) {
-#pragma unroll
-          for (int j = 0; j < 32; ++j) f[j] = act_call(f[j], EA_ACT_SILU);
-        } else if (p.act == EA_ACT_GELU) {
-#pragma unroll
-          for (int j = 0; j < 32; ++j) f[j] = gelu_erf_f(f[j]);
-        }
-        if (p.out_scale != 1.0f) {
-#pragma unroll
-          for (int j = 0; j < 32; ++j) f[j] *= p.out_scale;
-        }
-#pragma unroll
-        for (int q = 0; q < 4; ++q) {
-          const int slot = lane * 8 + ((half * 4 + q) ^ (lane & 7));
-          if (has_res) {
-            const uint4 rc = stg2[slot];
-            const float2 a = ea_unpack2(rc.x), b = ea_unpack2(rc.y), cc = ea_unpack2(rc.z), d = ea_unpack2(rc.w);
-            f[q * 8 + 0] += a.x; f[q * 8 + 1] += a.y; f[q * 8 + 2] += b.x; f[q * 8 + 3] += b.y;
-            f[q * 8 + 4] += cc.x; f[q * 8 + 5] += cc.y; f[q * 8 + 6] += d.x; f[q * 8 + 7] += d.y;
-          }
-          stg[slot] = make_uint4(ea_pack2(f[q * 8 + 0], f[q * 8 + 1]), ea_pack2(f[q * 8 + 2], f[q * 8 + 3]),
-                                 ea_pack2(f[q * 8 + 4], f[q * 8 + 5]), ea_pack2(f[q * 8 + 6], f[q * 8 + 7]));
-        }
-        if (p.rowstats_out) {
-          float s0 = 0.f, s1 = 0.f, q0 = 0.f, q1 = 0.f;
-#pragma unroll
-          for (int j = 0; j < 32; j += 2) {
-            s0 += f[j]; q0 = fmaf(f[j], f[j], q0);
-            s1 += f[j + 1]; q1 = fmaf(f[j + 1], f[j + 1], q1);
-          }
-          if (ri.ok && n_first < p.N) p.rowstats_out[(size_t)(n_first >> 5) * p.M + ri.m] = make_float2(s0 + s1, q0 + q1);
-        }
-        if (half == 1 || c + 32 >= BN)
-          stage_flush(stg, lane, p.out, p.ldo, p.out2, p.ldo2, ri.m, ri.ok, n_first - half * 32,
-                      half == 1 ? 8 : 4, p.N, lin_m0, p.M);
-      }
-    } else if (p.splits == 1) {
-      if (geglu) {
-        for (int c = wg * 32; c < half_bn; c += 64) {
-          uint32_t xv[32], gv[32];
-          acc_ld32(accs, ACC_LD, r, c, xv);
-          acc_ld32(accs, ACC_LD, r, half_bn + c, gv);
-          float fx[32], fg[32];
-#pragma unroll
-          for (int j = 0; j < 32; ++j) { fx[j] = __uint_as_float(xv[j]); fg[j] = __uint_as_float(gv[j]); }
-          uint4 o[4];
-          epilogue_geglu32(cbt, half_bn, c, fx, fg, o, ln, ln_r, ln_nm);
-          stage_put32(stg, lane, 0, o);
-          if (lin_m0 >= 0)
-            stage_flush32(stg, lane, p.out, p.ldo, (ncol0 >> 1) + c, p.N >> 1, lin_m0, p.M);
-          else
-            stage_flush(stg, lane, p.out, p.ldo, nullptr, 0, ri.m, ri.ok, (ncol0 >> 1) + c, 4, p.N >> 1, lin_m0, p.M);
-        }
-      } else {
-        for (int c = wg * 32; c < BN; c += 64) {
-          uint32_t v[32];
-          acc_ld32(accs, ACC_LD, r, c, v);
-          float f[32];
-#pragma unroll
-          for (int j = 0; j < 32; ++j) f[j] = __uint_as_float(v[j]);
-          epilogue_chunk32(p, ri, ncol0 + c, f);
-          __syncwarp();
-        }
-      }
+    };
+    if constexpr (R::split_epi) {
+      mma_tile();
+      __syncwarp();
+      if (lane == 0) mbar_arrive(acc_full);
     } else {
-      const int tile_id = tn * m_tiles + tm;
-      float* wtile = p.ws + (size_t)tile_id * p.splits * (BM * BN);
-      float* mine = wtile + (size_t)zsplit * (BM * BN);
-      for (int c = wg * 32; c < BN; c += 64) {
-        uint32_t v[32];
-        acc_ld32(accs, ACC_LD, r, c, v);
-        float4* dst = reinterpret_cast<float4*>(mine + (size_t)r * BN + c);
-#pragma unroll
-        for (int j = 0; j < 8; ++j)
-          __stcg(dst + j, make_float4(__uint_as_float(v[4 * j]), __uint_as_float(v[4 * j + 1]),
-                                      __uint_as_float(v[4 * j + 2]), __uint_as_float(v[4 * j + 3])));
-      }
-      __threadfence();
-      epi_bar_sync();
-      int* cnt = p.cnt + 2 * tile_id;
-      bool take_all = false;
-      volatile int* flag = reinterpret_cast<volatile int*>(cbt);
-      if (p.no_spin) {
-        if (et == 0) *flag = atomicAdd(cnt, 1);
-        epi_bar_sync();
-        take_all = *flag == p.splits - 1;
-        epi_bar_sync();
-      } else {
-        if (et == 0) {
-          atomicAdd(cnt, 1);
-          uint32_t spins = 0;
-          while (ld_acquire_gpu(cnt) < p.splits) {
-            __nanosleep(40);
-            if (++spins > (1u << 24)) { asm volatile("trap;"); }
-          }
-        }
-        epi_bar_sync();
-      }
-      __threadfence();
-      if (!p.no_spin || take_all) {
-        const int chunks = geglu ? (half_bn >> 5) : (BN >> 5);
-        const int units = BM * chunks;
-        const int u0 = take_all ? 0 : (int)(((long long)units * zsplit) / p.splits);
-        const int u1 = take_all ? units : (int)(((long long)units * (zsplit + 1)) / p.splits);
-        const int segs = geglu ? 2 : 1;
-        const int ustride = segs * 32 + 4;
-        float* stage_f = accs;
-        const size_t split_stride = (size_t)BM * BN;
-        for (int ub = u0; ub < u1; ub += EPI_THREADS) {
-          const int nu = min(EPI_THREADS, u1 - ub);
-          const int nvec4 = nu * segs * 8;
-          for (int idx = et; idx < nvec4; idx += EPI_THREADS) {
-            const int ul = idx / (segs * 8);
-            const int rem = idx - ul * (segs * 8);
-            const int seg = rem >> 3, q = rem & 7;
-            const int u = ub + ul;
-            const int rr = u & (BM - 1);
-            const int c = ((u >> 7) << 5) + seg * half_bn * (geglu ? 1 : 0);
-            const float4* src = reinterpret_cast<const float4*>(wtile + (size_t)rr * BN + c) + q;
-            float4 acc = make_float4(0.f, 0.f, 0.f, 0.f);
-            int sidx = 0;
-            for (; sidx + 4 <= p.splits; sidx += 4) {
-              float4 v0 = __ldcg(src + (size_t)(sidx + 0) * (split_stride >> 2));
-              float4 v1 = __ldcg(src + (size_t)(sidx + 1) * (split_stride >> 2));
-              float4 v2 = __ldcg(src + (size_t)(sidx + 2) * (split_stride >> 2));
-              float4 v3 = __ldcg(src + (size_t)(sidx + 3) * (split_stride >> 2));
-              acc.x += v0.x; acc.y += v0.y; acc.z += v0.z; acc.w += v0.w;
-              acc.x += v1.x; acc.y += v1.y; acc.z += v1.z; acc.w += v1.w;
-              acc.x += v2.x; acc.y += v2.y; acc.z += v2.z; acc.w += v2.w;
-              acc.x += v3.x; acc.y += v3.y; acc.z += v3.z; acc.w += v3.w;
-            }
-            for (; sidx < p.splits; ++sidx) {
-              float4 v0 = __ldcg(src + (size_t)sidx * (split_stride >> 2));
-              acc.x += v0.x; acc.y += v0.y; acc.z += v0.z; acc.w += v0.w;
-            }
-            *reinterpret_cast<float4*>(stage_f + ul * ustride + seg * 32 + q * 4) = acc;
-          }
-          epi_bar_sync();
-          if (et < nu) {
-            const int u = ub + et;
-            const int rr = u & (BM - 1);
-            const int c = (u >> 7) << 5;
-            RowInfo r2 = row_info(p, tm, rr);
-            const float4* sp = reinterpret_cast<const float4*>(stage_f + et * ustride);
-            float f[32];
-#pragma unroll
-            for (int j = 0; j < 8; ++j) {
-              float4 v = sp[j];
-              f[4 * j] = v.x; f[4 * j + 1] = v.y; f[4 * j + 2] = v.z; f[4 * j + 3] = v.w;
-            }
-            if (geglu) {
-              float fg[32];
-#pragma unroll
-              for (int j = 0; j < 8; ++j) {
-                float4 v = sp[8 + j];
-                fg[4 * j] = v.x; fg[4 * j + 1] = v.y; fg[4 * j + 2] = v.z; fg[4 * j + 3] = v.w;
-              }
-              epilogue_geglu32_direct(p, r2, ncol0, half_bn, c, f, fg);
-            } else {
-              epilogue_chunk32(p, r2, ncol0 + c, f);
-            }
-          }
-          epi_bar_sync();
-        }
-        epi_bar_sync();
-        if (et == 0) {
-          if (take_all) {
-            cnt[0] = 0;
-          } else {
-            int old = atomicAdd(cnt + 1, 1);
-            if (old == p.splits - 1) {
-              cnt[0] = 0;
-              cnt[1] = 0;
-            }
-          }
-        }
-      }
-    }
-    fence_proxy_async();
-    __syncwarp();
-    if (lane == 0) mbar_arrive(epi_done);
+      gemm_epilogue<BN>(p, tm, tn, zsplit, m_tiles, cb + (it & 1) * 512, accs,
+                        reinterpret_cast<uint4*>(stg_base + (warp - EPI_WARPS) * 4096), wg, wq, lane,
+                        threadIdx.x - EPI_THREADS, mma_tile);
+      fence_proxy_async();
+      __syncwarp();
+      if (lane == 0) mbar_arrive(acc_empty);
+    }
   }
 }
 #undef EA_GEMM_TILE
@@ -916,7 +995,8 @@
         cost = (double)waves * (PL_START + kbps * t_kb + PL_SPLIT_COL * BN) + PL_SPLIT_FIX +
                3.0 * (BM * BN * 4.0) / 25.0 + 150.0 * splits;
       }
-      if (cost < best.cost) best = {BN, st, splits, kbps, 1, cost};
+      if (cost < best.cost)
+        best = {BN, gemm_fit_stages(BN, st, gemm_split_epi(BN, kbps, splits)), splits, kbps, 1, cost};
     }
   }
   return best;
@@ -1071,23 +1151,25 @@
   return EA_OK;
 }
 
-template <int BN, int NG>
+template <int BN, int NG, bool SPLIT>
 static cudaError_t launch_gemm(const GemmLaunch<NG>& L, int grid, int smem_bytes, int tiles_per_group, int m_tiles,
                                int n_groups, cudaStream_t stream, int& rc) {
   static int cache[EA_MAX_DEV];
-  if ((rc = set_max_smem(ea_gemm_kernel<BN, NG>, smem_bytes, cache[ea_dev()]))) return cudaSuccess;
-  return ea_launch(ea_gemm_kernel<BN, NG>, dim3((unsigned)grid), dim3(GEMM_THREADS), (size_t)smem_bytes, stream, L,
-                   tiles_per_group, m_tiles, n_groups);
+  if ((rc = set_max_smem(ea_gemm_kernel<BN, NG, SPLIT>, smem_bytes, cache[ea_dev()]))) return cudaSuccess;
+  return ea_launch(ea_gemm_kernel<BN, NG, SPLIT>, dim3((unsigned)grid), dim3(GEMM_THREADS), (size_t)smem_bytes, stream,
+                   L, tiles_per_group, m_tiles, n_groups);
 }
 
 template <int NG>
-static cudaError_t launch_gemm_bn(int BN, const GemmLaunch<NG>& L, int grid, int smem_bytes, int tiles_per_group,
-                                  int m_tiles, int n_groups, cudaStream_t stream, int& rc) {
+static cudaError_t launch_gemm_bn(int BN, bool split, const GemmLaunch<NG>& L, int grid, int smem_bytes,
+                                  int tiles_per_group, int m_tiles, int n_groups, cudaStream_t stream, int& rc) {
   switch (BN) {
-    case 32: return launch_gemm<32, NG>(L, grid, smem_bytes, tiles_per_group, m_tiles, n_groups, stream, rc);
-    case 64: return launch_gemm<64, NG>(L, grid, smem_bytes, tiles_per_group, m_tiles, n_groups, stream, rc);
-    case 128: return launch_gemm<128, NG>(L, grid, smem_bytes, tiles_per_group, m_tiles, n_groups, stream, rc);
-    default: return launch_gemm<256, NG>(L, grid, smem_bytes, tiles_per_group, m_tiles, n_groups, stream, rc);
+    case 32: return launch_gemm<32, NG, true>(L, grid, smem_bytes, tiles_per_group, m_tiles, n_groups, stream, rc);
+    case 64: return launch_gemm<64, NG, true>(L, grid, smem_bytes, tiles_per_group, m_tiles, n_groups, stream, rc);
+    case 128:
+      return split ? launch_gemm<128, NG, true>(L, grid, smem_bytes, tiles_per_group, m_tiles, n_groups, stream, rc)
+                   : launch_gemm<128, NG, false>(L, grid, smem_bytes, tiles_per_group, m_tiles, n_groups, stream, rc);
+    default: return launch_gemm<256, NG, false>(L, grid, smem_bytes, tiles_per_group, m_tiles, n_groups, stream, rc);
   }
 }
 
@@ -1109,9 +1191,9 @@
   const int G = n_groups;
   const long long ws_floats =
       (a->workspace && a->workspace_bytes > 65536 && !ln_any) ? (a->workspace_bytes - 65536) / 4 : 0;
-  const bool persist = a->force_persistent > 0;
+  const bool force_persist = a->force_persistent > 0;
   const bool has_res = a->residual != nullptr;
-  GemmPlan plan = plan_gemm(m_tiles, a->N, nkb, a->act, persist ? 0 : ws_floats, sm_count(), has_res, G);
+  GemmPlan plan = plan_gemm(m_tiles, a->N, nkb, a->act, force_persist ? 0 : ws_floats, sm_count(), has_res, G);
   if (a->force_bn > 0 || a->force_stages > 0 || a->force_splits > 0) {
     if (a->force_bn > 0) plan.BN = a->force_bn;
     const int sb = BM * BK * 2 + plan.BN * BK * 2;
@@ -1120,7 +1202,7 @@
     if (plan.stages * sb > GEMM_SMEM_RING) plan.stages = GEMM_SMEM_RING / sb;
     if (plan.stages > nkb) plan.stages = nkb < 2 ? 2 : nkb;
     if (a->force_bn > 0 || a->force_splits > 0) { plan.splits = 1; plan.kbps = nkb; }
-    if (a->force_splits > 1 && !persist) {
+    if (a->force_splits > 1 && !force_persist) {
       plan.kbps = (nkb + a->force_splits - 1) / a->force_splits;
       plan.splits = (nkb + plan.kbps - 1) / plan.kbps;
     }
@@ -1136,10 +1218,12 @@
     return EA_ERR_SHAPE;
   if (plan.splits > 1 && !a->no_spin && tiles * G * plan.splits > (long long)sm_count()) return EA_ERR_SHAPE;
 
+  const bool split_epi = gemm_split_epi(BN, plan.kbps, plan.splits);
   int stages = plan.stages;
   if (stages > 8) stages = 8;
   if (stages < 2) stages = 2;
-  const int smem_bytes = gemm_region_bytes(BN, stages) + (2 * stages + 2) * 8 + 2 * 2 * 256 * 4 + 1024;
+  stages = gemm_fit_stages(BN, stages, split_epi);
+  const int smem_bytes = gemm_smem_bytes(BN, stages, split_epi);
   const long long tiles_per_group = tiles * plan.splits;
   for (int g = 0; g < G; ++g) {
     GemmKParams& p = L.g[g].p;
@@ -1162,6 +1246,7 @@
   if (m_tiles > 64)
     for (int g = 0; g < G; ++g) L.g[g].p.b_policy = 0ull;
   const long long total = tiles_per_group * G;
+  const bool persist = force_persist || (a->force_persistent == 0 && plan.splits == 1 && split_epi);
   const int grid = (int)(persist && total > sm_count() ? sm_count() : total);
   for (int g = 0; g < G; ++g)
     L.g[g].p.pf_ctas = grid < sm_count() ? grid : sm_count();
@@ -1171,9 +1256,9 @@
   if (G == 1) {
     GemmLaunch<1> L1;
     L1.g[0] = L.g[0];
-    le = launch_gemm_bn<1>(BN, L1, grid, smem_bytes, (int)tiles_per_group, m_tiles, G, stream, rc);
+    le = launch_gemm_bn<1>(BN, split_epi, L1, grid, smem_bytes, (int)tiles_per_group, m_tiles, G, stream, rc);
   } else {
-    le = launch_gemm_bn<GEMM_MAX_GROUPS>(BN, L, grid, smem_bytes, (int)tiles_per_group, m_tiles, G, stream, rc);
+    le = launch_gemm_bn<GEMM_MAX_GROUPS>(BN, split_epi, L, grid, smem_bytes, (int)tiles_per_group, m_tiles, G, stream, rc);
   }
   if (rc) return rc;
   ea_count_launch();
```

Measured after the change: 1.683 (median of 6 runs). 4.0% higher.
